# utiasASRL/mm_masking

Hardware: AMD Instinct MI355X
Metric: scan-pairs/s (mask-CNN + 10-iter dICP fwd+bwd) (higher is better)
Workload: dtype bf16; 1 GPU; BASELINE configs[2]: train_icp_weights step fwd+bwd, batch=32 per GPU, 10 dICP iters, point-to-plane Huber, dim=2; 400x3360 polar radar -> GO-CFAR + peaks + polar->Cartesian 640x640 -> U-Net (hand-written NHWC bf16 MFMA kernels, fp32 masters) -> dICP (fp32 points, fp64 normal equations) -> rot+trans+mask_pts loss -> Adam; batch_per_gpu=32, global_batch=32, scan_pts_pad=5120, map_pts=20000, map_pts_pad=20480, icp_iters=10, parallelism=dp1, scene_density=survey (SURVEY.md 8d: 3 500-5 000 valid scan points of 5 120)

## Files before the change

include/mmk.h:

```cpp
#ifndef MMK_H_
#define MMK_H_

#include <stddef.h>
#include <stdint.h>

#ifdef __cplusplus
extern "C" {
#endif

#define MMK_VERSION 502

#define MMK_OK 0
#define MMK_ERR_ARG (-1)
#define MMK_ERR_HIP (-2)
#define MMK_ERR_WORKSPACE (-3)

#define MMK_ICP_PT2PT 0
#define MMK_ICP_PT2PL 1

#define MMK_NN_BRUTE 0
#define MMK_NN_GRID 1

#define MMK_LOSS_NONE 0
#define MMK_LOSS_CAUCHY 1
// ... 72 lines not shown
int mmk_pose_loss_fwd(const float *T_pred , int32_t B, float *out2, void *stream);
int mmk_pose_loss_bwd(const float *T_pred, int32_t B, const float *g_rot, const float *g_trans,
                      float *grad_T , void *stream);
size_t mmk_bce_ws_bytes(void);
int mmk_bce_mean_fwd(const float *x, const float *target, int64_t n, void *ws, size_t ws_bytes,
                     float *out, void *stream);
int mmk_bce_mean_bwd(const float *x, const float *target, int64_t n, const float *grad_out,
                     float *grad_x, void *stream);

int mmk_pose_loss_gt_fwd(const float *T_pred , const float *T_gt , int32_t B, float *out2, void *stream);
int mmk_pose_loss_gt_bwd(const float *T_pred, const float *T_gt, int32_t B, const float *g_rot, const float *g_trans,
                         float *grad_T , void *stream);
int mmk_val_metric(const float *T_pred , const float *T_gt , int32_t B, float *out3, void *stream);
size_t mmk_fft_threshold_ws_bytes(int32_t B);
int mmk_fft_threshold_mask(const float *fft, int32_t B, int64_t hw, void *ws, size_t ws_bytes, float *mask_out,
                           void *stream);
int mmk_bce_fft_threshold_fwd(const float *x, const float *fft, int32_t B, int64_t hw, void *ws, size_t ws_bytes,
                              float *thr_out , float *out, void *stream);
int mmk_bce_fft_threshold_bwd(const float *x, const float *fft, int32_t B, int64_t hw, const float *thr ,
                              const float *grad_out, float *grad_x, void *stream);


int mmk_cfar_mask(const float *raw, int32_t B, int32_t A, int32_t R, int32_t w2,
                  int32_t guard, int32_t mincol, int32_t maxcol, float a_thresh,
                  float b_thresh, int32_t diff, float steep_fact, float *mask,
                  void *stream);

int mmk_cfar_mask_bwd(const float *raw, const float *grad_mask , int32_t B, int32_t A, int32_t R, int32_t w2,
                      int32_t guard, int32_t mincol, int32_t maxcol, float a_thresh, float b_thresh, float steep_fact,
                      float *grad_raw , void *stream);

size_t mmk_extract_peaks_workspace_bytes(int32_t B, int32_t A, int32_t R, int32_t max_pts);
int mmk_extract_peaks(const float *mask, int32_t B, int32_t A, int32_t R, float res,
                      const float *azimuths , const float *times ,
                      const float *T_ab, int32_t diff, float steep_fact, int32_t max_pts,
                      float *out_pc, int32_t *out_count, void *workspace,
                      size_t workspace_bytes, void *stream);
size_t mmk_extract_peaks_bwd_workspace_bytes(int32_t B, int32_t A, int32_t R, int32_t max_pts);
int mmk_extract_peaks_bwd(const float *mask, int32_t B, int32_t A, int32_t R, float res, const float *azimuths ,
                          const float *T_ab, int32_t diff, float steep_fact, int32_t max_pts,
                          const float *grad_pc , float *grad_mask , void *workspace,
                          size_t workspace_bytes, void *stream);

int mmk_polar_to_cart(const float *polar, const float *azimuths ,
                      const float *range_grid, const float *angle_grid, int32_t B,
                      int32_t A, int32_t R, int32_t W, float radar_resolution,
                      int32_t interpolate_crossover, int32_t fix_wobble, float *cart,
                      void *stream);
int mmk_polar_to_cart_pair(const float *polar, const float *polar2, const float *azimuths,
                           const float *range_grid, const float *angle_grid, int32_t B, int32_t A,
                           int32_t R, int32_t W, float radar_resolution, int32_t interpolate_crossover,
                           int32_t fix_wobble, float *cart, float *cart2, void *stream);

int mmk_cart_to_polar(const double *cart, const double *sin_az, const double *cos_az, const double *range_coords,
                      int32_t B, int32_t A, int32_t R, int32_t H, int32_t W, double cart_resolution, double *polar,
                      void *stream);

size_t mmk_polar_to_cart_bwd_ws_bytes(int32_t B, int32_t A, int32_t R, int32_t W);
int mmk_polar_to_cart_bwd(const float *grad_cart , const float *azimuths , const float *range_grid,
                          const float *angle_grid, int32_t B, int32_t A, int32_t R, int32_t W, float radar_resolution,
                          int32_t interpolate_crossover, int32_t fix_wobble, float *grad_polar , void *ws,
                          size_t ws_bytes, void *stream);

size_t mmk_cart_to_polar_bwd_ws_bytes(int32_t B, int32_t A, int32_t R, int32_t H, int32_t W);
int mmk_cart_to_polar_bwd(const double *grad_polar , const double *sin_az, const double *cos_az,
                          const double *range_coords, int32_t B, int32_t A, int32_t R, int32_t H, int32_t W,
                          double radar_resolution, double cart_resolution, double *grad_cart , void *ws,
                          size_t ws_bytes, void *stream);

int mmk_mask_polar_scan(const float *scan , const float *mask_cart , const double *sin_az,
                        const double *cos_az, const double *range_coords, int32_t B, int32_t A, int32_t R, int32_t H,
                        int32_t W, double cart_resolution, float *out , void *stream);

size_t mmk_mask_polar_scan_bwd_ws_bytes(int32_t B, int32_t A, int32_t R, int32_t H, int32_t W);
int mmk_mask_polar_scan_bwd(const float *grad_out , const float *scan , const float *mask_cart ,
                            const double *sin_az, const double *cos_az, const double *range_coords, int32_t B, int32_t A,
                            int32_t R, int32_t H, int32_t W, double radar_resolution, double cart_resolution,
                            float *grad_scan , float *grad_mask , void *ws, size_t ws_bytes,
                            void *stream);

int mmk_sample_weights_fwd(const float *mask , const float *pc ,
                           int32_t B, int32_t N, int32_t pc_cols, int32_t H, int32_t W,
                           int32_t cart_pixel_width, float cart_resolution,
                           float *weights , void *stream);
size_t mmk_sample_weights_bwd_ws_bytes(int32_t B, int32_t N);
int mmk_sample_weights_bwd(const float *grad_weights , const float *pc, int32_t B,
                           int32_t N, int32_t pc_cols, int32_t H, int32_t W,
                           int32_t cart_pixel_width, float cart_resolution, float *grad_mask,
                           void *ws, size_t ws_bytes, void *stream);
int mmk_sample_weights_bwd_pc(const float *grad_weights , const float *mask , const float *pc,
                              int32_t B, int32_t N, int32_t pc_cols, int32_t H, int32_t W,
                              int32_t cart_pixel_width, float cart_resolution, float *grad_pc, void *stream);

int mmk_host_read_rows(const char *path, int64_t header_bytes, int32_t rows, int32_t row_bytes, int32_t col0,
                       int32_t ncols, int32_t roll, void *dst);
typedef struct mmk_read_job {
    const char *path;
    int64_t header_bytes;
    int32_t rows, row_bytes, col0, ncols, roll, reserved;
    void *dst;
} mmk_read_job;
int mmk_host_read_rows_batch(const mmk_read_job *jobs, int32_t n_jobs, int32_t threads);
int mmk_u8_to_float(const void *in , const float *lut256, int64_t n, float *out, void *stream);

int mmk_weight_stats(const float *weights , const float *pc , int32_t B, int32_t N,
                     int32_t pc_cols, float *partial, float *out, void *stream);

int mmk_bev_raster(const float *pc , int32_t B, int32_t M, int32_t pc_cols,
                   int32_t W, float cart_resolution, float *bev , void *stream);

typedef struct {
    const void *x1;
    const void *x2;
    int32_t C1, C2;
    const void *wpack;
    const float *bias;
    void *y1;
    const void *relu_src1;
    int32_t O1, accumulate1;
    float scale1;
    void *y2;
    const void *relu_src2;
    int32_t O2, accumulate2;
    float scale2;
    int32_t B, H, W;
    int32_t relu;
    float leaky_slope;
    float drop_p;
    uint32_t seed;
    void *pool_y;
    void *pool_arg;
} mmk_conv_desc;

int32_t mmk_conv3x3_pool_fusable(int32_t cin, int32_t cout, int32_t B, int32_t H, int32_t W);

size_t mmk_conv3x3_packed_elems(int32_t cout, int32_t cin, int32_t transposed);
int mmk_conv3x3_pack_weights(const float *W, int32_t cout, int32_t cin, int32_t transposed,
                             void *packed, void *stream);
int mmk_conv3x3_pack_weights_batch(int32_t n, const float *const *W, const int32_t *cout, const int32_t *cin,
                                   int32_t transposed, void *const *packed, void *stream);
int mmk_conv3x3(const mmk_conv_desc *d, void *stream);
int32_t mmk_conv3x3_wgrad_slices(int32_t cout, int32_t cin, int32_t c1, int32_t B, int32_t H, int32_t W);
int mmk_conv3x3_wgrad_partial(const void *x1, const void *x2, int32_t C1, int32_t C2, const void *g, int32_t cout,
                              int32_t B, int32_t H, int32_t W, float *partials, int32_t accumulate, void *stream);

int mmk_conv_bwd_fused(const void *x, const void *g, const void *wpack_t, float scale, int32_t B, int32_t H, int32_t W,
                       int32_t C, void *dx, float *partials, int32_t accumulate, void *stream);

int mmk_conv8x16_bwd_fused(const void *x, const void *g, const void *wpack_t, float scale, int32_t B, int32_t H, int32_t W,
                           void *dx, float *partials, int32_t accumulate, void *stream);

int mmk_conv16x8_bwd_fused(const void *x1, const void *x2, const void *g, const void *wpack_t, float scale, int32_t B, int32_t H,
                           int32_t W, void *dx1, void *dx2, float *partials, int32_t accumulate, void *stream);
int mmk_conv3x3_wgrad_unpack_batch(int32_t n, const float *const *src, const int32_t *slices, const int32_t *cout,
                                   const int32_t *cin, float *const *dW, float *const *db, void *stream);

int mmk_channel_minmax(const float *x , int32_t B, int32_t C, int64_t hw, float *part,
                       float *pre , float *minmax , void *stream);
int mmk_channel_meanstd(const float *x , int32_t B, int32_t C, int64_t hw, double *part,
                        float *pre , void *stream);
int mmk_conv_first(const float *x, int32_t cin, const float *W, const float *bias, const float *pre,
                   int32_t B, int32_t H, int32_t Wd, float leaky_slope, void *y, void *stream);
size_t mmk_conv_first_wgrad_ws_bytes(int32_t cin);
int mmk_conv_first_wgrad(const float *x, int32_t cin, const void *g, const float *pre, int32_t B,
                         int32_t H, int32_t Wd, float *dW, float *db, float *ws, size_t ws_bytes, void *stream);
#define MMK_NORM_NONE 0
#define MMK_NORM_MINMAX 1
#define MMK_NORM_STANDARDIZE 2
size_t mmk_conv_first_dgrad_ws_bytes(int32_t cin);
int mmk_conv_first_dgrad(const void *g, int32_t cin, const float *W, const float *x , const float *pre ,
                         const float *minmax , int32_t B, int32_t H, int32_t Wd, float *grad_x, void *ws ,
                         size_t ws_bytes, void *stream);
int mmk_input_norm_bwd(float *grad_x, const float *x, int32_t cin, const float *pre, const float *minmax ,
                       int32_t mode, int32_t B, int32_t H, int32_t Wd, const void *ws, size_t ws_bytes, void *stream);

int mmk_maxpool2_fwd(const void *x, int32_t B, int32_t H, int32_t W, int32_t C, void *y, void *stream);
int mmk_maxpool2_bwd(const void *d, const void *gy, int32_t B, int32_t H, int32_t W, int32_t C, float scale,
                     float leaky_slope, void *gz, void *stream);
int mmk_maxpool2_fwd_arg(const void *x, int32_t B, int32_t H, int32_t W, int32_t C, void *y, void *arg, void *stream);
int mmk_maxpool2_bwd_arg(const void *arg, const void *gy, int32_t B, int32_t H, int32_t W, int32_t C, float scale,
                         void *gz, void *stream);

int mmk_upsample_fwd(const void *x, int32_t B, int32_t Hs, int32_t Ws, int32_t C, int32_t Ho, int32_t Wo, void *y,
                     void *stream);
int mmk_upsample_bwd(const void *gy, int32_t B, int32_t Hs, int32_t Ws, int32_t C, int32_t Ho, int32_t Wo,
                     const void *relu_src, float scale, float leaky_slope, void *gx, void *stream);

#define MMK_FINAL_BWD_WS_FLOATS 16384
int mmk_final_fwd(const void *x, const float *w, const float *bias, int64_t npix, float *mask, void *stream);
int mmk_final_bwd(const void *x, const float *w, const float *mask, const float *gmask, int64_t npix, float scale,
                  float leaky_slope, void *gx, float *dW, float *db, float *ws, void *stream);
int mmk_mask_normalize(const float *mask , int32_t B, int64_t npix_per, float *part,
                       float *mask_n, float *amax, void *stream);
int mmk_final_bwd_normalized(const void *x, const float *w, const float *mask, const float *mask_n,
                             const float *amax, const float *gmask_n, int32_t B, int64_t npix_per,
                             float scale, float leaky_slope, float *part, float *coef, void *gx, float *dW,
                             float *db, float *ws, void *stream);

int mmk_bn_forward_stats(const void *a, int64_t npix, int32_t C, const float *gamma, const float *beta, float eps,
                         float momentum, float *running_mean, float *running_var, float *part, float *stat,
                         float *affine, void *stream);
int mmk_bn_apply(const void *a, int64_t npix, int32_t C, const float *affine, float drop_p, uint32_t seed, void *y,
                 void *stream);
int mmk_bn_backward(const void *gd, const void *d, float drop_scale, const void *a, int64_t npix, int32_t C,
                    const float *stat, const float *affine, const float *gamma, float leaky_slope, int32_t accumulate,
                    float *part, float *coef, float *dgamma, float *dbeta, void *gz, void *stream);

typedef struct {
    int32_t B, H, W, cin;
    const float *x;
    const float *pre;
    const float *const *params;
    float drop_p;
    uint32_t seed;
    float leaky_slope;
    int32_t norm;
    void *workspace;
    size_t workspace_bytes;
    float *mask;
    int32_t keep_full_res;
} mmk_unet_desc;

size_t mmk_unet_workspace_bytes(int32_t B, int32_t H, int32_t W, int32_t cin);
size_t mmk_unet_scratch_bytes(int32_t B, int32_t H, int32_t W, int32_t cin);
int mmk_unet_forward(const mmk_unet_desc *d, void *stream);
int mmk_unet_backward(const mmk_unet_desc *d, const float *gmask, float *const *grads, void *scratch,
                      size_t scratch_bytes, void *stream);
#define MMK_UNET_GRAD_BUCKETS 3
int32_t mmk_unet_grad_bucket(int32_t bucket, int32_t *first_param, int32_t *n_params);
int mmk_unet_backward_buckets(const mmk_unet_desc *d, const float *gmask, float *const *grads, void *scratch,
                              size_t scratch_bytes, void *const *bucket_events, void *stream);
int mmk_unet_backward_input(const mmk_unet_desc *d, const float *gmask, float *const *grads, float *grad_x, int32_t norm_mode,
                            const float *minmax, void *scratch, size_t scratch_bytes, void *const *bucket_events, void *stream);
int mmk_unet_tensor(int32_t B, int32_t H, int32_t W, int32_t cin, int32_t id, size_t *offset, int32_t *h,
                    int32_t *w, int32_t *c);

#ifdef __cplusplus
}
#endif
#endif
```

mm_masking_amd/_lib.py:

```python
import ctypes
import os
import sys
import subprocess

import torch

_HERE = os.path.dirname(os.path.abspath(__file__))
_ROOT = os.path.dirname(_HERE)
SO_PATH = os.environ.get("MMK_LIB", os.path.join(_HERE, "libmmk_hip.so"))
SOURCES = ["mmk_api.hip", "mmk_icp.hip", "mmk_radar.hip", "mmk_unet.hip", "mmk_unet_driver.hip", "mmk_loader.hip", "mmk_loss.hip"]

_lib = None

c_f32p = ctypes.c_void_p
c_vp = ctypes.c_void_p


class MmkError(RuntimeError):
    pass


class ReadJob(ctypes.Structure):
    _fields_ = [("path", ctypes.c_char_p), ("header_bytes", ctypes.c_int64), ("rows", ctypes.c_int32),
                ("row_bytes", ctypes.c_int32), ("col0", ctypes.c_int32), ("ncols", ctypes.c_int32), ("roll", ctypes.c_int32),
                ("reserved", ctypes.c_int32), ("dst", ctypes.c_void_p)]


class IcpParams(ctypes.Structure):
    _fields_ = [("B", ctypes.c_int32), ("N", ctypes.c_int32), ("M", ctypes.c_int32),
                ("tgt_cols", ctypes.c_int32), ("dim", ctypes.c_int32), ("icp_type", ctypes.c_int32),
                ("loss", ctypes.c_int32), ("loss_k", ctypes.c_float), ("trim_dist", ctypes.c_float),
                ("tolerance", ctypes.c_float), ("max_iter", ctypes.c_int32), ("save_state", ctypes.c_int32),
                ("check_every", ctypes.c_int32), ("nn_method", ctypes.c_int32)]


class ConvDesc(ctypes.Structure):
    _fields_ = [("x1", ctypes.c_void_p), ("x2", ctypes.c_void_p), ("C1", ctypes.c_int32), ("C2", ctypes.c_int32),
                ("wpack", ctypes.c_void_p), ("bias", ctypes.c_void_p),
                ("y1", ctypes.c_void_p), ("relu_src1", ctypes.c_void_p), ("O1", ctypes.c_int32),
                ("accumulate1", ctypes.c_int32), ("scale1", ctypes.c_float),
                ("y2", ctypes.c_void_p), ("relu_src2", ctypes.c_void_p), ("O2", ctypes.c_int32),
                ("accumulate2", ctypes.c_int32), ("scale2", ctypes.c_float),
                ("B", ctypes.c_int32), ("H", ctypes.c_int32), ("W", ctypes.c_int32), ("relu", ctypes.c_int32),
                ("leaky_slope", ctypes.c_float), ("drop_p", ctypes.c_float), ("seed", ctypes.c_uint32), ("pool_y", ctypes.c_void_p),
                ("pool_arg", ctypes.c_void_p)]


class UNetDesc(ctypes.Structure):
    _fields_ = [("B", ctypes.c_int32), ("H", ctypes.c_int32), ("W", ctypes.c_int32), ("cin", ctypes.c_int32),
                ("x", ctypes.c_void_p), ("pre", ctypes.c_void_p), ("params", ctypes.POINTER(ctypes.c_void_p)),
                ("drop_p", ctypes.c_float), ("seed", ctypes.c_uint32), ("leaky_slope", ctypes.c_float), ("norm", ctypes.c_int32),
                ("workspace", ctypes.c_void_p), ("workspace_bytes", ctypes.c_size_t), ("mask", ctypes.c_void_p),
                ("keep_full_res", ctypes.c_int32)]


FINAL_BWD_WS_FLOATS = 16384
NORM_MODES = {None: 0, "none": 0, "minmax": 1, "standardize": 2}
ICP_TYPES = {"pt2pt": 0, "pt2pl": 1}
LOSSES = {None: 0, "none": 0, "l2": 0, "cauchy": 1, "huber": 2}
NN_METHODS = {"brute": 0, "grid": 1}


def build(verbose=False):
    from concurrent.futures import ThreadPoolExecutor
    csrc = os.path.join(_HERE, "csrc")
    srcs = [os.path.join(csrc, s) for s in SOURCES]
    common = [os.path.join(csrc, "mmk_common.h"), os.path.join(csrc, "mmk_unet_shared.h"), os.path.join(_ROOT, "include", "mmk.h")]
    incs = [os.path.join(csrc, f) for f in sorted(os.listdir(csrc)) if f.endswith(".inc")]
    extra = {"mmk_unet.hip": incs, "mmk_loader.hip": incs}
    objdir = os.path.join(csrc, "_obj")
    os.makedirs(objdir, exist_ok=True)
    hipcc = os.environ.get("HIPCC", "/opt/rocm/bin/hipcc")
    flags = ["--offload-arch=gfx950", "-O3", "-std=c++17", "-fPIC", "-ffp-contract=off", "-I", os.path.join(_ROOT, "include")]
    per_file = {"mmk_unet.hip": ["-mllvm", "-amdgpu-mfma-vgpr-form"]}
    jobs, objs = [], []
    for src in srcs:
        obj = os.path.join(objdir, os.path.basename(src)[:-4] + ".o")
        objs.append(obj)
        deps = [src] + common + extra.get(os.path.basename(src), []) + [os.path.abspath(__file__)]
        if not (os.path.exists(obj) and all(os.path.getmtime(obj) >= os.path.getmtime(d) for d in deps)):
            jobs.append([hipcc] + flags + per_file.get(os.path.basename(src), []) + ["-c", src, "-o", obj])
    if not jobs and os.path.exists(SO_PATH) and all(os.path.getmtime(SO_PATH) >= os.path.getmtime(o) for o in objs):
        return SO_PATH

    def run(cmd):
        if verbose:
            print(" ".join(cmd), flush=True)
        try:
            subprocess.check_call(cmd)
        except subprocess.CalledProcessError:
            plain = [c for c in cmd if c not in sum(per_file.values(), [])]
            if len(plain) == len(cmd):
                raise
            print("libmmk_hip: retrying without %s" % " ".join(sorted(set(cmd) - set(plain))), file=sys.stderr, flush=True)
            subprocess.check_call(plain)
    with ThreadPoolExecutor(max_workers=max(1, min(len(jobs), os.cpu_count() or 1))) as ex:
        list(ex.map(run, jobs))
    run([hipcc, "--offload-arch=gfx950", "-shared", "-fPIC", "-o", SO_PATH] + objs)
    return SO_PATH


def _declare(lib):
    i32, f32, sz = ctypes.c_int32, ctypes.c_float, ctypes.c_size_t
    P = ctypes.POINTER(IcpParams)
    sig = {
        "mmk_version": (ctypes.c_int, []),
        "mmk_last_error": (ctypes.c_char_p, []),
        "mmk_icp_workspace_bytes": (sz, [P]),
        "mmk_icp_forward": (ctypes.c_int, [P] + [c_vp] * 10 + [c_vp, sz, ctypes.POINTER(ctypes.c_int), c_vp]),
        "mmk_icp_backward": (ctypes.c_int, [P] + [c_vp] * 11 + [c_vp, sz, c_vp]),
        "mmk_icp_backward_points_workspace_bytes": (sz, [P, i32]),
        "mmk_icp_backward_points": (ctypes.c_int, [P] + [c_vp] * 13 + [c_vp, sz, c_vp]),
        "mmk_icp_status": (ctypes.c_int, [P, c_vp, sz, c_vp, c_vp]),
        "mmk_pose_loss_fwd": (ctypes.c_int, [c_vp, i32, c_vp, c_vp]),
        "mmk_pose_loss_bwd": (ctypes.c_int, [c_vp, i32, c_vp, c_vp, c_vp, c_vp]),
        "mmk_bce_ws_bytes": (sz, []),
        "mmk_bce_mean_fwd": (ctypes.c_int, [c_vp, c_vp, ctypes.c_int64, c_vp, sz, c_vp, c_vp]),
        "mmk_bce_mean_bwd": (ctypes.c_int, [c_vp, c_vp, ctypes.c_int64, c_vp, c_vp, c_vp]),
        "mmk_pose_loss_gt_fwd": (ctypes.c_int, [c_vp, c_vp, i32, c_vp, c_vp]),
        "mmk_pose_loss_gt_bwd": (ctypes.c_int, [c_vp, c_vp, i32, c_vp, c_vp, c_vp, c_vp]),
        "mmk_val_metric": (ctypes.c_int, [c_vp, c_vp, i32, c_vp, c_vp]),
        "mmk_fft_threshold_ws_bytes": (sz, [i32]),
        "mmk_fft_threshold_mask": (ctypes.c_int, [c_vp, i32, ctypes.c_int64, c_vp, sz, c_vp, c_vp]),
        "mmk_bce_fft_threshold_fwd": (ctypes.c_int, [c_vp, c_vp, i32, ctypes.c_int64, c_vp, sz, c_vp, c_vp, c_vp]),
        "mmk_bce_fft_threshold_bwd": (ctypes.c_int, [c_vp, c_vp, i32, ctypes.c_int64, c_vp, c_vp, c_vp, c_vp]),
        "mmk_icp_partials_count": (sz, [P]),
        "mmk_icp_accumulate": (ctypes.c_int, [P] + [c_vp] * 8 + [c_vp]),
        "mmk_icp_solve_update": (ctypes.c_int, [P] + [c_vp] * 7 + [c_vp]),
        "mmk_nn_padded_m": (i32, [i32]),
        "mmk_pack_target": (ctypes.c_int, [c_vp, i32, i32, i32, i32, c_vp, c_vp]),
        "mmk_nn_workspace_bytes": (sz, [i32, i32, i32, i32]),
        "mmk_nn_search": (ctypes.c_int, [c_vp, c_vp, c_vp, i32, i32, i32, i32, c_vp, c_vp, c_vp, sz, c_vp]),
        "mmk_nn_profile_begin": (ctypes.c_int, [i32]),
        "mmk_nn_profile_end": (ctypes.c_int, [ctypes.POINTER(ctypes.c_float), i32, ctypes.POINTER(ctypes.c_int32)]),
        "mmk_conv3x3_packed_elems": (sz, [i32, i32, i32]),
        "mmk_conv3x3_pack_weights": (ctypes.c_int, [c_vp, i32, i32, i32, c_vp, c_vp]),
        "mmk_conv3x3_pack_weights_batch": (ctypes.c_int, [i32, c_vp, c_vp, c_vp, i32, c_vp, c_vp]),
        "mmk_conv3x3": (ctypes.c_int, [ctypes.POINTER(ConvDesc), c_vp]),
        "mmk_conv3x3_wgrad_unpack_batch": (ctypes.c_int, [i32, c_vp, c_vp, c_vp, c_vp, c_vp, c_vp, c_vp]),
        "mmk_conv3x3_wgrad_slices": (i32, [i32, i32, i32, i32, i32, i32]),
        "mmk_conv3x3_wgrad_partial": (ctypes.c_int, [c_vp, c_vp, i32, i32, c_vp, i32, i32, i32, i32, c_vp, i32, c_vp]),
        "mmk_conv_bwd_fused": (ctypes.c_int, [c_vp, c_vp, c_vp, ctypes.c_float, i32, i32, i32, i32, c_vp, c_vp, i32, c_vp]),
        "mmk_conv8x16_bwd_fused": (ctypes.c_int, [c_vp, c_vp, c_vp, ctypes.c_float, i32, i32, i32, c_vp, c_vp, i32, c_vp]),
        "mmk_conv16x8_bwd_fused": (ctypes.c_int, [c_vp, c_vp, c_vp, c_vp, ctypes.c_float, i32, i32, i32, c_vp, c_vp, c_vp, i32, c_vp]),
        "mmk_conv3x3_pool_fusable": (ctypes.c_int32, [i32, i32, i32, i32, i32]),
        "mmk_channel_minmax": (ctypes.c_int, [c_vp, i32, i32, ctypes.c_int64, c_vp, c_vp, c_vp, c_vp]),
        "mmk_channel_meanstd": (ctypes.c_int, [c_vp, i32, i32, ctypes.c_int64, c_vp, c_vp, c_vp]),
        "mmk_conv_first": (ctypes.c_int, [c_vp, i32, c_vp, c_vp, c_vp, i32, i32, i32, f32, c_vp, c_vp]),
        "mmk_conv_first_wgrad_ws_bytes": (sz, [i32]),
        "mmk_conv_first_wgrad": (ctypes.c_int, [c_vp, i32, c_vp, c_vp, i32, i32, i32, c_vp, c_vp, c_vp, sz, c_vp]),
        "mmk_conv_first_dgrad_ws_bytes": (sz, [i32]),
        "mmk_conv_first_dgrad": (ctypes.c_int, [c_vp, i32, c_vp, c_vp, c_vp, c_vp, i32, i32, i32, c_vp, c_vp, sz, c_vp]),
        "mmk_input_norm_bwd": (ctypes.c_int, [c_vp, c_vp, i32, c_vp, c_vp, i32, i32, i32, i32, c_vp, sz, c_vp]),
        "mmk_maxpool2_fwd": (ctypes.c_int, [c_vp, i32, i32, i32, i32, c_vp, c_vp]),
        "mmk_maxpool2_bwd": (ctypes.c_int, [c_vp, c_vp, i32, i32, i32, i32, f32, f32, c_vp, c_vp]),
        "mmk_maxpool2_fwd_arg": (ctypes.c_int, [c_vp, i32, i32, i32, i32, c_vp, c_vp, c_vp]),
        "mmk_maxpool2_bwd_arg": (ctypes.c_int, [c_vp, c_vp, i32, i32, i32, i32, f32, c_vp, c_vp]),
        "mmk_upsample_fwd": (ctypes.c_int, [c_vp, i32, i32, i32, i32, i32, i32, c_vp, c_vp]),
        "mmk_upsample_bwd": (ctypes.c_int, [c_vp, i32, i32, i32, i32, i32, i32, c_vp, f32, f32, c_vp, c_vp]),
        "mmk_final_fwd": (ctypes.c_int, [c_vp, c_vp, c_vp, ctypes.c_int64, c_vp, c_vp]),
        "mmk_final_bwd": (ctypes.c_int, [c_vp, c_vp, c_vp, c_vp, ctypes.c_int64, f32, f32, c_vp, c_vp, c_vp, c_vp, c_vp]),
        "mmk_mask_normalize": (ctypes.c_int, [c_vp, i32, ctypes.c_int64, c_vp, c_vp, c_vp, c_vp]),
        "mmk_final_bwd_normalized": (ctypes.c_int, [c_vp, c_vp, c_vp, c_vp, c_vp, c_vp, i32, ctypes.c_int64, f32, f32, c_vp, c_vp,
                                                    c_vp, c_vp, c_vp, c_vp, c_vp]),
        "mmk_bn_forward_stats": (ctypes.c_int, [c_vp, ctypes.c_int64, i32, c_vp, c_vp, f32, f32, c_vp, c_vp, c_vp, c_vp, c_vp, c_vp]),
        "mmk_bn_apply": (ctypes.c_int, [c_vp, ctypes.c_int64, i32, c_vp, f32, ctypes.c_uint32, c_vp, c_vp]),
        "mmk_bn_backward": (ctypes.c_int, [c_vp, c_vp, f32, c_vp, ctypes.c_int64, i32, c_vp, c_vp, c_vp, f32, i32, c_vp, c_vp, c_vp,
                                           c_vp, c_vp, c_vp]),
        "mmk_unet_workspace_bytes": (sz, [i32, i32, i32, i32]),
        "mmk_unet_scratch_bytes": (sz, [i32, i32, i32, i32]),
        "mmk_unet_forward": (ctypes.c_int, [ctypes.POINTER(UNetDesc), c_vp]),
        "mmk_unet_backward": (ctypes.c_int, [ctypes.POINTER(UNetDesc), c_vp, ctypes.POINTER(ctypes.c_void_p), c_vp, sz, c_vp]),
        "mmk_unet_backward_buckets": (ctypes.c_int, [ctypes.POINTER(UNetDesc), c_vp, ctypes.POINTER(ctypes.c_void_p), c_vp, sz,
                                                     ctypes.POINTER(ctypes.c_void_p), c_vp]),
        "mmk_unet_backward_input": (ctypes.c_int, [ctypes.POINTER(UNetDesc), c_vp, ctypes.POINTER(ctypes.c_void_p), c_vp, i32, c_vp,
                                                   c_vp, sz, ctypes.POINTER(ctypes.c_void_p), c_vp]),
        "mmk_unet_grad_bucket": (i32, [i32, ctypes.POINTER(i32), ctypes.POINTER(i32)]),
        "mmk_unet_tensor": (ctypes.c_int, [i32, i32, i32, i32, i32, ctypes.POINTER(sz), ctypes.POINTER(i32), ctypes.POINTER(i32),
                                           ctypes.POINTER(i32)]),
        "mmk_cfar_mask": (ctypes.c_int, [c_vp, i32, i32, i32, i32, i32, i32, i32, f32, f32, i32, f32, c_vp, c_vp]),
        "mmk_cfar_mask_bwd": (ctypes.c_int, [c_vp, c_vp, i32, i32, i32, i32, i32, i32, i32, f32, f32, f32, c_vp, c_vp]),
        "mmk_extract_peaks_workspace_bytes": (sz, [i32, i32, i32, i32]),
        "mmk_extract_peaks_bwd_workspace_bytes": (sz, [i32, i32, i32, i32]),
        "mmk_extract_peaks_bwd": (ctypes.c_int, [c_vp, i32, i32, i32, f32, c_vp, c_vp, i32, f32, i32, c_vp, c_vp, c_vp, sz, c_vp]),
        "mmk_extract_peaks": (ctypes.c_int, [c_vp, i32, i32, i32, f32, c_vp, c_vp, c_vp, i32, f32, i32, c_vp, c_vp,
                                             c_vp, sz, c_vp]),
        "mmk_polar_to_cart": (ctypes.c_int, [c_vp, c_vp, c_vp, c_vp, i32, i32, i32, i32, f32, i32, i32, c_vp, c_vp]),
        "mmk_polar_to_cart_pair": (ctypes.c_int, [c_vp, c_vp, c_vp, c_vp, c_vp, i32, i32, i32, i32, f32, i32, i32, c_vp, c_vp,
                                                  c_vp]),
        "mmk_cart_to_polar": (ctypes.c_int, [c_vp, c_vp, c_vp, c_vp, i32, i32, i32, i32, i32, ctypes.c_double, c_vp, c_vp]),
        "mmk_polar_to_cart_bwd_ws_bytes": (sz, [i32, i32, i32, i32]),
        "mmk_polar_to_cart_bwd": (ctypes.c_int, [c_vp, c_vp, c_vp, c_vp, i32, i32, i32, i32, f32, i32, i32, c_vp, c_vp, sz, c_vp]),
        "mmk_cart_to_polar_bwd_ws_bytes": (sz, [i32, i32, i32, i32, i32]),
        "mmk_cart_to_polar_bwd": (ctypes.c_int, [c_vp, c_vp, c_vp, c_vp, i32, i32, i32, i32, i32, ctypes.c_double, ctypes.c_double,
                                                 c_vp, c_vp, sz, c_vp]),
        "mmk_mask_polar_scan": (ctypes.c_int, [c_vp, c_vp, c_vp, c_vp, c_vp, i32, i32, i32, i32, i32, ctypes.c_double, c_vp, c_vp]),
        "mmk_mask_polar_scan_bwd_ws_bytes": (sz, [i32, i32, i32, i32, i32]),
        "mmk_mask_polar_scan_bwd": (ctypes.c_int, [c_vp, c_vp, c_vp, c_vp, c_vp, c_vp, i32, i32, i32, i32, i32, ctypes.c_double,
                                                   ctypes.c_double, c_vp, c_vp, c_vp, sz, c_vp]),
        "mmk_sample_weights_fwd": (ctypes.c_int, [c_vp, c_vp, i32, i32, i32, i32, i32, i32, f32, c_vp, c_vp]),
        "mmk_host_read_rows": (ctypes.c_int, [ctypes.c_char_p, ctypes.c_int64, i32, i32, i32, i32, i32, c_vp]),
        "mmk_host_read_rows_batch": (ctypes.c_int, [ctypes.POINTER(ReadJob), i32, i32]),
        "mmk_u8_to_float": (ctypes.c_int, [c_vp, c_vp, ctypes.c_int64, c_vp, c_vp]),
        "mmk_sample_weights_bwd_ws_bytes": (sz, [i32, i32]),
        "mmk_sample_weights_bwd": (ctypes.c_int, [c_vp, c_vp, i32, i32, i32, i32, i32, i32, f32, c_vp, c_vp, sz, c_vp]),
        "mmk_sample_weights_bwd_pc": (ctypes.c_int, [c_vp, c_vp, c_vp, i32, i32, i32, i32, i32, i32, f32, c_vp, c_vp]),
        "mmk_weight_stats": (ctypes.c_int, [c_vp, c_vp, i32, i32, i32, c_vp, c_vp, c_vp]),
        "mmk_bev_raster": (ctypes.c_int, [c_vp, i32, i32, i32, i32, f32, c_vp, c_vp]),
    }
    for name, (res, args) in sig.items():
        fn = getattr(lib, name)
        fn.restype = res
        fn.argtypes = args
    return sig


EXPORTED = None


def lib():
    global _lib, EXPORTED
    if _lib is None:
        if not os.path.exists(SO_PATH):
            raise MmkError("libmmk_hip.so is not built: run `python -c 'import __graft_entry__ as g; g.build()'` "
                           "(hipcc --offload-arch=gfx950).  The HIP path has no CPU fallback.")
        try:
            loaded = ctypes.CDLL(SO_PATH)
        except OSError as e:
            raise MmkError("cannot load %s: %s" % (SO_PATH, e)) from e
        EXPORTED = _declare(loaded)
        _lib = loaded
    return _lib


def check(rc):
    if rc != 0:
        raise MmkError("libmmk_hip: %s (code %d)" % (lib().mmk_last_error().decode(errors="replace"), rc))


def stream_ptr(device=None):
    if device is not None:
        idx = device.index if isinstance(device, torch.device) else int(device)
        if idx is not None and idx != torch.cuda.current_device():
            raise MmkError("tensors live on cuda:%d but the current HIP device is cuda:%d: call torch.cuda.set_device() "
                           "(one process per GPU) or wrap the call in `with torch.cuda.device(...)`"
                           % (idx, torch.cuda.current_device()))
    return ctypes.c_void_p(torch.cuda.current_stream(device).cuda_stream)


def ptr(t, dtype=None, name="tensor"):
    if t is None:
        return ctypes.c_void_p(0)
    if not t.is_cuda:
        raise MmkError("%s must live on a HIP device (got %s); the kernels have no CPU path" % (name, t.device))
    if dtype is not None and t.dtype != dtype:
        raise MmkError("%s must be %s (got %s)" % (name, dtype, t.dtype))
    if not t.is_contiguous():
        raise MmkError("%s must be contiguous" % name)
    return ctypes.c_void_p(t.data_ptr())


def dev_f32(t, device):
    return t.detach().to(device=device, dtype=torch.float32).contiguous()
```

mm_masking_amd/csrc/mmk_unet.hip:

```cpp
#include <math.h>
#include <stdlib.h>

#include <algorithm>
#include <type_traits>

#include "mmk_common.h"
#include "mmk_unet_shared.h"

namespace {

using namespace mmku;

__device__ __forceinline__ unsigned cvt_pk_bf16(float lo, float hi)
{
    unsigned r;
    asm("v_cvt_pk_bf16_f32 %0, %1, %2" : "=v"(r) : "v"(lo), "v"(hi));
    return r;
}
__device__ __forceinline__ unsigned pk_relu_bf16(unsigned x)
{
    unsigned r;
    asm("v_pk_max_i16 %0, %1, 0" : "=v"(r) : "v"(x));
    return r;
}
// ... 1419 lines not shown
        t_end = min(total_tiles, (xcd + 1) * per_xcd);
    } else {
        t_first = blockIdx.x; t_step = gridDim.x; t_end = total_tiles;
    }
    const int adv_tx = t_step % tiles_x, adv_ty = (t_step / tiles_x) % tiles_y, adv_b = t_step / tpi;
    int ld_b = t_first / tpi, ld_ty = (t_first % tpi) / tiles_x, ld_tx = t_first % tiles_x;
    if (t_first < t_end) load_tile(ld_b, ld_ty, ld_tx);
    for (int t = t_first; t < t_end; t += t_step) {
        __syncthreads();
        store_tile();
        __syncthreads();
        {
            if (t + t_step < t_end) {
                ld_tx += adv_tx;
                const int cx = ld_tx >= tiles_x ? 1 : 0;
                ld_tx -= cx ? tiles_x : 0;
                ld_ty += adv_ty + cx;
                const int cy = ld_ty >= tiles_y ? 1 : 0;
                ld_ty -= cy ? tiles_y : 0;
                ld_b += adv_b + cy;
            }
            load_tile(ld_b, ld_ty, ld_tx);
        }
        i32x2 fa[2][2 * MT], fb[2][2 * NTW];
#define WG_ISSUE(R, BUF)                                                                                 \
    {                                                                                                    \
        _Pragma("unroll") for (int m = 0; m < MT; ++m) {                                                 \
            fa[BUF][2 * m] = (m == 0) ? tr_read_o<((R) * TW * PG) * 2>(g_ad)                             \
                           : (m == 1) ? tr_read_o<((R) * TW * PG + 16) * 2>(g_ad)                        \
                           : (m == 2) ? tr_read_o<((R) * TW * PG + 32) * 2>(g_ad)                        \
                                      : tr_read_o<((R) * TW * PG + 48) * 2>(g_ad);                       \
            fa[BUF][2 * m + 1] = (m == 0) ? tr_read_o<((R) * TW * PG + 16 * PG) * 2>(g_ad)                \
                               : (m == 1) ? tr_read_o<((R) * TW * PG + 16 + 16 * PG) * 2>(g_ad)           \
                               : (m == 2) ? tr_read_o<((R) * TW * PG + 32 + 16 * PG) * 2>(g_ad)           \
                                          : tr_read_o<((R) * TW * PG + 48 + 16 * PG) * 2>(g_ad);          \
        }                                                                                                \
        _Pragma("unroll") for (int n = 0; n < NTW; ++n) {                                                \
            fb[BUF][2 * n] = tr_read_o<((R) * WT * PK) * 2>(b_ad[n]);                                    \
            fb[BUF][2 * n + 1] = tr_read_o<((R) * WT * PK + 16 * PK) * 2>(b_ad[n]);                       \
        }                                                                                                \
    }
#define WG_CONSUME(BUF)                                                                                  \
    {                                                                                                    \
        _Pragma("unroll") for (int m = 0; m < MT; ++m) {                                                 \
            const bf16x8 af = frag_from(fa[BUF][2 * m], fa[BUF][2 * m + 1]);                             \
             \
             \
            _Pragma("unroll") for (int n = 0; n < NTW; ++n)                                              \
                acc[m][n] = __builtin_amdgcn_mfma_f32_16x16x32_bf16(af, frag_from(fb[BUF][2 * n], fb[BUF][2 * n + 1]), acc[m][n], 0, 0, 0); \
            accb[m] = __builtin_amdgcn_mfma_f32_16x16x32_bf16(af, ones, accb[m], 0, 0, 0);               \
        }                                                                                                \
    }
#define WG_STEP(R)                                                                                       \
    {                                                                                                    \
        asm volatile("s_waitcnt lgkmcnt(0)" ::: "memory");                                               \
        __builtin_amdgcn_sched_barrier(0);                                                               \
        if ((R) + 1 < TH) WG_ISSUE(((R) + 1 < TH ? (R) + 1 : 0), ((R) + 1) & 1);                         \
        __builtin_amdgcn_sched_barrier(0);                                                               \
        WG_CONSUME((R) & 1);                                                                             \
    }
        WG_ISSUE(0, 0);
        WG_STEP(0) WG_STEP(1) WG_STEP(2) WG_STEP(3) WG_STEP(4) WG_STEP(5) WG_STEP(6) WG_STEP(7)
        static_assert(TH == 8, "WG_STEP expansion above covers 8 tile rows");
#undef WG_STEP
#undef WG_CONSUME
#undef WG_ISSUE
    }

    const size_t pstride = (size_t)9 * a.COUT * a.CIN + a.COUT;
#pragma unroll
    for (int m = 0; m < MT; ++m) {
#pragma unroll
        for (int rr = 0; rr < 4; ++rr) {
            const int co = group * CM + m * 16 + g4 * 4 + rr;
            if (co >= a.COUT) continue;
#pragma unroll
            for (int n = 0; n < NTW; ++n) {
                const int nt = wv + 4 * n;
                if (nt >= NTT) continue;
                int tap, ci;
                if (CK >= 16) {
                    tap = nt / (CK / 16);
                    ci = chunk * CK + (nt % (CK / 16)) * 16 + i16;
                } else {
                    tap = 2 * nt + (i16 >> 3);
                    ci = i16 & 7;
                }
                if (tap < 9) {
                    float *d = a.partials + (size_t)blockIdx.x * pstride + ((size_t)tap * a.COUT + co) * a.CIN + ci;
                    *d = a.acc_partials ? *d + acc[m][n][rr] : acc[m][n][rr];
                }
            }
            if (wv == 0 && chunk == 0 && i16 == 0) {
                float *d = a.partials + (size_t)blockIdx.x * pstride + (size_t)9 * a.COUT * a.CIN + co;
                *d = a.acc_partials ? *d + accb[m][rr] : accb[m][rr];
            }
        }
    }
}

template <int CK, int CM, bool G8>
int wgrad_spatial(int cout, int cin, int B, int H, int W)
{
    const size_t smem = ((size_t)(HT * WT + 8) * wg_pitch(CK) + (size_t)(TH * TW + 8) * wg_pitch(G8 ? 8 : CM)) * sizeof(bf16);
    static int per_cu[64] = {};
    int dev = 0;
    if (hipGetDevice(&dev) != hipSuccess) return -1;
    if (per_cu[dev & 63] == 0) {
        if (smem > 64 * 1024 &&
            hipFuncSetAttribute((const void *)conv3x3_wgrad_kernel<CK, CM, G8>, hipFuncAttributeMaxDynamicSharedMemorySize, (int)smem) != hipSuccess)
            return -1;
        int nblk = 0;
        if (hipOccupancyMaxActiveBlocksPerMultiprocessor(&nblk, conv3x3_wgrad_kernel<CK, CM, G8>, CONV_THREADS, smem) != hipSuccess)
            return -1;
        const int cap = (CK <= 16 && CM == 16) ? 4 : 8;
        per_cu[dev & 63] = nblk < 1 ? 1 : (nblk > cap ? cap : nblk);
    }
    const int tiles = ((W + TW - 1) / TW) * ((H + TH - 1) / TH) * B;
    const int chunks = cin / CK, groups = (cout + CM - 1) / CM;
    int spatial = (256 * per_cu[dev & 63]) / (chunks * groups);
    spatial = spatial < 1 ? 1 : (spatial > tiles ? tiles : spatial);
    return spatial >= 8 ? (spatial & ~7) : spatial;
}

template <int CK, int CM, bool G8>
int launch_wgrad(const WgradArgs &a, hipStream_t st)
{
    const size_t smem = ((size_t)(HT * WT + 8) * wg_pitch(CK) + (size_t)(TH * TW + 8) * wg_pitch(G8 ? 8 : CM)) * sizeof(bf16);
    const int spatial = wgrad_spatial<CK, CM, G8>(a.COUT, a.CIN, a.B, a.H, a.W);
    if (spatial < 1) {
        mmk::set_error("mmk_conv3x3_wgrad: occupancy query failed");
        return MMK_ERR_HIP;
    }
    const int chunks = a.CIN / CK, groups = (a.COUT + CM - 1) / CM;
    hipLaunchKernelGGL((conv3x3_wgrad_kernel<CK, CM, G8>), dim3(spatial, chunks, groups), dim3(CONV_THREADS), smem, st, a);
    MMK_LAUNCH_CHECK();
    return MMK_OK;
}


struct BwdFusedArgs {
    const bf16 *x, *x2;
    const bf16 *g;
    const bf16 *wpack_t;
    bf16 *dx, *dx2;
    float scale;
    int masked;
    int accumulate_dx;
    int B, H, W;
    float *partials;
    int acc_partials;
};

template <int CX, int CG>
__global__ __launch_bounds__(CONV_THREADS) void conv_bwd_fused_kernel(const BwdFusedArgs a)
{
    static_assert((CX == 8 || CX == 16) && (CG == 8 || CG == 16), "thin layers");
    constexpr int NTT = CX == 8 ? 5 : 9;
    constexpr int NTW = (NTT + 3) / 4;
    constexpr int NS = CG == 8 ? 3 : 5;
    constexpr int NT = 4;
    constexpr int GX = CX / 8, GG = CG / 8;
    __shared__ __attribute__((aligned(16))) bf16 x_tile[(HT * WT + 8) * CX];
    __shared__ __attribute__((aligned(16))) bf16 g_tile[(HT * WT + 8) * CG];
    __shared__ __attribute__((aligned(16))) bf16 w_lds[NS * 64 * 8];

    const int tid = threadIdx.x, lane = tid & 63;
    const int wv = __builtin_amdgcn_readfirstlane(tid >> 6);
    const int tiles_x = (a.W + TW - 1) / TW, tiles_y = (a.H + TH - 1) / TH;
    const int tpi = tiles_x * tiles_y;
    const int total_tiles = tpi * a.B;
    const int i16 = lane & 15, g4 = lane >> 4, q = i16 >> 2, pp = i16 & 3;
    const bool split = a.x2 != nullptr;

    f32x4 acc[NTW], accb = {0.f, 0.f, 0.f, 0.f};
#pragma unroll
    for (int n = 0; n < NTW; ++n) acc[n] = (f32x4){0.f, 0.f, 0.f, 0.f};
    bf16x8 ones;
#pragma unroll
    for (int j = 0; j < 8; ++j) ones[j] = (bf16)1.0f;
    unsigned b_ad[NTW];
#pragma unroll
    for (int n = 0; n < NTW; ++n) {
        const int nt = wv + 4 * n;
        int tap = CX == 8 ? 2 * nt + (pp >> 1) : nt;
        const int col = CX == 8 ? 4 * (pp & 1) : 4 * pp;
        tap = tap > 8 ? 8 : tap;
        const int ty = tap / 3, tx = tap % 3;
        b_ad[n] = lds_addr(x_tile) + (unsigned)((((ty * WT) + 4 * g4 + q + tx) * CX + col) * 2);
    }
    const unsigned g_ad = lds_addr(g_tile) + (unsigned)(((WT + 1 + 4 * g4 + q) * CG + 4 * pp) * 2);

    int d_lane[NS];
#pragma unroll
    for (int ks = 0; ks < NS; ++ks) {
        int tap = CG == 8 ? 4 * ks + (lane >> 4) : 2 * ks + (lane >> 5);
        const int ch = CG == 8 ? 0 : 8 * ((lane >> 4) & 1);
        tap = tap > 8 ? 8 : tap;
        d_lane[ks] = ((2 * wv + tap / 3) * WT + (lane & 15) + tap % 3) * CG + ch;
    }
    const int n8 = lane >> 4;
    const int lrow8 = 2 * wv + (n8 >> 1), lcol8 = (n8 & 1) * 16 + (lane & 15);
    const int lpix8 = lrow8 * a.W + lcol8;
    const int s_off8 = ((lrow8 + 1) * WT + lcol8 + 1) * CX;
    int o_pix[NT], s_off[NT];
#pragma unroll
    for (int n = 0; n < NT; ++n) {
        const int r = 2 * wv + (n >> 1), c = (n & 1) * 16 + (lane & 15);
        o_pix[n] = r * a.W + c;
        s_off[n] = ((r + 1) * WT + c + 1) * CX + (lane >> 4) * 4;
    }
    bf16 *const o_base = (a.dx2 != nullptr) ? ((lane >> 5) ? a.dx2 : a.dx) + ((lane >> 4) & 1) * 4 : a.dx + (lane >> 4) * 4;
    const int o_stride = (a.dx2 != nullptr) ? 8 : 16;
    for (int i = tid; i < NS * 64; i += CONV_THREADS) reinterpret_cast<u32x4 *>(w_lds)[i] = reinterpret_cast<const u32x4 *>(a.wpack_t)[i];

    constexpr int NX = HT * WT * GX, NG = HT * WT * GG;
    constexpr int RX = (NX + CONV_THREADS - 1) / CONV_THREADS, RG = (NG + CONV_THREADS - 1) / CONV_THREADS;
    u32x4 rx[RX], rg[RG];
    auto load_tile = [&](int b, int tyi, int txi) {
        int tv = tid;
        asm volatile("" : "+v"(tv));
        const int tx0 = txi * TW, ty0 = tyi * TH;
        const int pix0 = (b * a.H + ty0) * a.W + tx0;
#pragma unroll
        for (int i = 0; i < RX; ++i) {
            int gi = tv + i * CONV_THREADS;
            gi = gi < NX ? gi : NX - 1;
            const int pix = gi / GX, half = gi % GX;
            const int dy = pix / WT - 1, dx = pix % WT - 1;
            const bool ok = (unsigned)(ty0 + dy) < (unsigned)a.H && (unsigned)(tx0 + dx) < (unsigned)a.W;
            const long po = pix0 + dy * a.W + dx;
            const bf16 *src = split ? (half ? a.x2 : a.x) + po * 8 : a.x + po * CX + half * 8;
            rx[i] = *(ok ? reinterpret_cast<const u32x4 *>(src) : &g_zero16);
        }
#pragma unroll
        for (int i = 0; i < RG; ++i) {
            int gi = tv + i * CONV_THREADS;
            gi = gi < NG ? gi : NG - 1;
            const int pix = gi / GG, gc = gi % GG;
            const int dy = pix / WT - 1, dx = pix % WT - 1;
            const bool ok = (unsigned)(ty0 + dy) < (unsigned)a.H && (unsigned)(tx0 + dx) < (unsigned)a.W;
            rg[i] = *(ok ? reinterpret_cast<const u32x4 *>(a.g + (long)(pix0 + dy * a.W + dx) * CG + gc * 8) : &g_zero16);
        }
    };
    auto store_tile = [&]() {
        int tv = tid;
        asm volatile("" : "+v"(tv));
#pragma unroll
        for (int i = 0; i < RX; ++i) {
            const int gi = tv + i * CONV_THREADS;
            if (gi < NX) *reinterpret_cast<u32x4 *>(x_tile + (size_t)gi * 8) = rx[i];
        }
#pragma unroll
        for (int i = 0; i < RG; ++i) {
            const int gi = tv + i * CONV_THREADS;
            if (gi < NG) *reinterpret_cast<u32x4 *>(g_tile + (size_t)gi * 8) = rg[i];
        }
    };

    int t_first, t_step, t_end;
    if ((gridDim.x & 7) == 0) {
        const int per_xcd = (total_tiles + 7) / 8;
        const int xcd = blockIdx.x & 7;
        t_first = xcd * per_xcd + ((int)blockIdx.x >> 3);
        t_step = (int)gridDim.x >> 3;
        t_end = min(total_tiles, (xcd + 1) * per_xcd);
    } else {
        t_first = blockIdx.x; t_step = gridDim.x; t_end = total_tiles;
    }
    const int adv_tx = t_step % tiles_x, adv_ty = (t_step / tiles_x) % tiles_y, adv_b = t_step / tpi;
    int ld_b = t_first / tpi, ld_ty = (t_first % tpi) / tiles_x, ld_tx = t_first % tiles_x;
    int cb = ld_b, cty = ld_ty, ctx = ld_tx;
    if (t_first < t_end) {
        load_tile(ld_b, ld_ty, ld_tx);
        store_tile();
    }
    __syncthreads();
    for (int t = t_first; t < t_end; t += t_step) {
        const int b = cb;
        const int tx0 = ctx * TW, ty0 = cty * TH;
        const int pix0 = (b * a.H + ty0) * a.W + tx0;
        const bool ok8 = (ty0 + lrow8) < a.H && (tx0 + lcol8) < a.W;
        u32x4 e8_acc = {0u, 0u, 0u, 0u};
        if constexpr (CX == 8) e8_acc = *((ok8 && a.accumulate_dx) ? reinterpret_cast<const u32x4 *>(a.dx + (long)(pix0 + lpix8) * 8) : &g_zero16);
        {
            if (t + t_step < t_end) {
                ld_tx += adv_tx;
                const int cx = ld_tx >= tiles_x ? 1 : 0;
                ld_tx -= cx ? tiles_x : 0;
                ld_ty += adv_ty + cx;
                const int cy = ld_ty >= tiles_y ? 1 : 0;
                ld_ty -= cy ? tiles_y : 0;
                ld_b += adv_b + cy;
            }
            load_tile(ld_b, ld_ty, ld_tx);
            cb = ld_b; cty = ld_ty; ctx = ld_tx;
        }
        i32x2 fa[2][2], fb[2][2 * NTW];
#define BF_ISSUE(R, BUF)                                                                     \
    {                                                                                        \
        fa[BUF][0] = tr_read_o<((R) * WT * CG) * 2>(g_ad);                                   \
        fa[BUF][1] = tr_read_o<((R) * WT * CG + 16 * CG) * 2>(g_ad);                         \
        _Pragma("unroll") for (int n = 0; n < NTW; ++n) {                                    \
            fb[BUF][2 * n] = tr_read_o<((R) * WT * CX) * 2>(b_ad[n]);                        \
            fb[BUF][2 * n + 1] = tr_read_o<((R) * WT * CX + 16 * CX) * 2>(b_ad[n]);          \
        }                                                                                    \
    }
#define BF_CONSUME(BUF)                                                                      \
    {                                                                                        \
        const bf16x8 af = frag_from(fa[BUF][0], fa[BUF][1]);                                 \
        _Pragma("unroll") for (int n = 0; n < NTW; ++n)                                      \
            acc[n] = __builtin_amdgcn_mfma_f32_16x16x32_bf16(af, frag_from(fb[BUF][2 * n], fb[BUF][2 * n + 1]), acc[n], 0, 0, 0); \
        accb = __builtin_amdgcn_mfma_f32_16x16x32_bf16(af, ones, accb, 0, 0, 0);             \
    }
#define BF_STEP(R)                                                                           \
    {                                                                                        \
        asm volatile("s_waitcnt lgkmcnt(0)" ::: "memory");                                   \
        __builtin_amdgcn_sched_barrier(0);                                                   \
        if ((R) + 1 < TH) BF_ISSUE(((R) + 1 < TH ? (R) + 1 : 0), ((R) + 1) & 1);             \
        __builtin_amdgcn_sched_barrier(0);                                                   \
        BF_CONSUME((R) & 1);                                                                 \
    }
        BF_ISSUE(0, 0);
        BF_STEP(0) BF_STEP(1) BF_STEP(2) BF_STEP(3) BF_STEP(4) BF_STEP(5) BF_STEP(6) BF_STEP(7)
        static_assert(TH == 8, "BF_STEP expansion above covers 8 tile rows");
#undef BF_STEP
#undef BF_CONSUME
#undef BF_ISSUE
        f32x4 dacc[NT];
#pragma unroll
        for (int n = 0; n < NT; ++n) dacc[n] = (f32x4){0.f, 0.f, 0.f, 0.f};
#pragma unroll
        for (int ks = 0; ks < NS; ++ks) {
            const bf16 *bl = g_tile + d_lane[ks];
            bf16x8 bf[NT];
#pragma unroll
            for (int n = 0; n < NT; ++n) bf[n] = *reinterpret_cast<const bf16x8 *>(bl + ((n >> 1) * WT + (n & 1) * 16) * CG);
            const bf16x8 af = *reinterpret_cast<const bf16x8 *>(w_lds + ((size_t)(ks * 64 + lane)) * 8);
#pragma unroll
            for (int n = 0; n < NT; ++n) dacc[n] = __builtin_amdgcn_mfma_f32_16x16x32_bf16(af, bf[n], dacc[n], 0, 0, 0);
        }
        u32x4 e8_src = {0u, 0u, 0u, 0u};
        bf16x4 e_src[NT];
        if constexpr (CX == 8) {
            e8_src = *reinterpret_cast<const u32x4 *>(x_tile + s_off8);
        } else {
#pragma unroll
            for (int n = 0; n < NT; ++n) e_src[n] = *reinterpret_cast<const bf16x4 *>(x_tile + s_off[n]);
        }
#pragma unroll
        for (int i = 0; i < RX; ++i) asm volatile("" : "+v"(rx[i]));
#pragma unroll
        for (int i = 0; i < RG; ++i) asm volatile("" : "+v"(rg[i]));
        if constexpr (CX == 8) {
            float v8[8];
#pragma unroll
            for (int r = 0; r < 4; ++r) {
                const auto s01 = __builtin_amdgcn_permlane16_swap(__float_as_uint(dacc[0][r]), __float_as_uint(dacc[1][r]), false, false);
                const auto s23 = __builtin_amdgcn_permlane16_swap(__float_as_uint(dacc[2][r]), __float_as_uint(dacc[3][r]), false, false);
                const auto lo = __builtin_amdgcn_permlane32_swap(s01[0], s23[0], false, false);
                const auto hi = __builtin_amdgcn_permlane32_swap(s01[1], s23[1], false, false);
                v8[r] = __uint_as_float(lo[0]);
                v8[4 + r] = __uint_as_float(hi[0]);
            }
            float sv[8], av[8];
            unpack8(e8_src, sv);
            unpack8(e8_acc, av);
#pragma unroll
            for (int r = 0; r < 8; ++r) {
                const float v = fmaxf(v8[r] + 0.f, -INFINITY);
                const float masked = (sv[r] > 0.f) ? v * a.scale : 0.f;
                v8[r] = masked + av[r];
            }
            u32x4 *dst8 = ok8 ? reinterpret_cast<u32x4 *>(a.dx + (long)(pix0 + lpix8) * 8) : reinterpret_cast<u32x4 *>(g_sink16);
            *dst8 = pack8(v8);
        } else {
#pragma unroll
            for (int n = 0; n < NT; ++n) {
                const bool okp = (ty0 + 2 * wv + (n >> 1)) < a.H && (tx0 + (n & 1) * 16 + (lane & 15)) < a.W;
                bf16x4 outv;
#pragma unroll
                for (int r = 0; r < 4; ++r) {
                    const float v = fmaxf(dacc[n][r] + 0.f, -INFINITY);
                    const float masked = ((float)e_src[n][r] > 0.f) ? v * a.scale : 0.f;
                    outv[r] = (bf16)(a.masked ? masked + 0.f : v);
                }
                bf16x4 *dst = okp ? reinterpret_cast<bf16x4 *>(o_base + (long)(pix0 + o_pix[n]) * o_stride) : reinterpret_cast<bf16x4 *>(g_sink16);
                *dst = outv;
            }
        }
        if (t + t_step >= t_end) break;
        __syncthreads();
        store_tile();
        __syncthreads();
    }

    constexpr size_t pstride = (size_t)9 * CG * CX + CG;
#pragma unroll
    for (int rr = 0; rr < 4; ++rr) {
        const int co = g4 * 4 + rr;
        if (co >= CG) continue;
#pragma unroll
        for (int n = 0; n < NTW; ++n) {
            const int nt = wv + 4 * n;
            if (nt >= NTT) continue;
            const int tap = CX == 8 ? 2 * nt + (i16 >> 3) : nt;
            const int ci = CX == 8 ? (i16 & 7) : i16;
            if (tap < 9) {
                float *d = a.partials + (size_t)blockIdx.x * pstride + ((size_t)tap * CG + co) * CX + ci;
                *d = a.acc_partials ? *d + acc[n][rr] : acc[n][rr];
            }
        }
        if (wv == 0 && i16 == 0) {
            float *d = a.partials + (size_t)blockIdx.x * pstride + (size_t)9 * CG * CX + co;
            *d = a.acc_partials ? *d + accb[rr] : accb[rr];
        }
    }
}

constexpr int WGD_THREADS = 512;

__global__ __launch_bounds__(WGD_THREADS) void conv3x3_wgrad_deep_kernel(const WgradArgs a)
{
    constexpr int CK = 64, CM = 64, PK = wg_pitch(64), PG = wg_pitch(64);
    extern __shared__ __attribute__((aligned(16))) unsigned char smem[];
    bf16 *x_tile = reinterpret_cast<bf16 *>(smem);
    bf16 *g_tile = x_tile + (HT * WT + 8) * PK;

    const int tid = threadIdx.x, lane = tid & 63;
    const int wv = __builtin_amdgcn_readfirstlane(tid >> 6);
    const int wm = wv >> 2, wc = wv & 3;
    const int chunk = blockIdx.y, group = blockIdx.z;
    const int tiles_x = (a.W + TW - 1) / TW, tiles_y = (a.H + TH - 1) / TH;
    const int tpi = tiles_x * tiles_y;
    const int total_tiles = tpi * a.B;
    const int i16 = lane & 15, g4 = lane >> 4, q = i16 >> 2, pp = i16 & 3;

    f32x4 acc[3][3][2];
    f32x4 accb[2];
#pragma unroll
    for (int m = 0; m < 2; ++m) {
        accb[m] = (f32x4){0.f, 0.f, 0.f, 0.f};
#pragma unroll
        for (int ty = 0; ty < 3; ++ty)
#pragma unroll
            for (int tx = 0; tx < 3; ++tx) acc[ty][tx][m] = (f32x4){0.f, 0.f, 0.f, 0.f};
    }
    bf16x8 ones;
#pragma unroll
    for (int j = 0; j < 8; ++j) ones[j] = (bf16)1.0f;

    const unsigned xb0 = lds_addr(x_tile) + (unsigned)(((4 * g4 + q) * PK + wc * 16 + 4 * pp) * 2);
    const unsigned gb0 = lds_addr(g_tile) + (unsigned)(((4 * g4 + q) * PG + wm * 32 + 4 * pp) * 2);

    constexpr int GPP = CK / 8;
    constexpr int NIN = HT * WT * GPP;
    constexpr int RIN = (NIN + WGD_THREADS - 1) / WGD_THREADS;
    constexpr int GPG = CM / 8;
    constexpr int NG = TH * TW * GPG;
    constexpr int RG = (NG + WGD_THREADS - 1) / WGD_THREADS;
    u32x4 rin[RIN], rg[RG];
    auto load_tile = [&](int b, int tyi, int txi) {
        int tv = tid;
        asm volatile("" : "+v"(tv));
        const int tx0 = txi * TW, ty0 = tyi * TH;
        const int c0 = chunk * CK;
        const bool in1 = c0 < a.C1;
        const bf16 *xb = in1 ? a.x1 : a.x2;
        const int xc = in1 ? a.C1 : a.C2, cb = in1 ? c0 : c0 - a.C1;
#pragma unroll
        for (int i = 0; i < RIN; ++i) {
            int gi = tv + i * WGD_THREADS;
            gi = gi < NIN ? gi : NIN - 1;
            const int pix = gi / GPP, gc = gi % GPP;
            const int yy = ty0 + pix / WT - 1, xx = tx0 + pix % WT - 1;
            const bool ok = yy >= 0 && yy < a.H && xx >= 0 && xx < a.W;
            const size_t p = ((size_t)b * a.H + yy) * a.W + xx;
            const u32x4 *sp = ok ? reinterpret_cast<const u32x4 *>(xb + p * xc + cb + gc * 8) : &g_zero16;
            rin[i] = *sp;
        }
#pragma unroll
        for (int i = 0; i < RG; ++i) {
            int gi = tv + i * WGD_THREADS;
            gi = gi < NG ? gi : NG - 1;
            const int pix = gi / GPG, gc = gi % GPG;
            const int yy = ty0 + pix / TW, xx = tx0 + pix % TW;
            const bool ok = yy < a.H && xx < a.W;
            const size_t p = ((size_t)b * a.H + yy) * a.W + xx;
            const u32x4 *sp = ok ? reinterpret_cast<const u32x4 *>(a.g + p * a.COUT + group * CM + gc * 8) : &g_zero16;
            rg[i] = *sp;
        }
    };
    auto store_tile = [&]() {
        int tv = tid;
        asm volatile("" : "+v"(tv));
#pragma unroll
        for (int i = 0; i < RIN; ++i) {
            const int gi = tv + i * WGD_THREADS;
            if (gi < NIN) *reinterpret_cast<u32x4 *>(x_tile + (size_t)(gi / GPP) * PK + (gi % GPP) * 8) = rin[i];
        }
#pragma unroll
        for (int i = 0; i < RG; ++i) {
            const int gi = tv + i * WGD_THREADS;
            if (gi < NG) *reinterpret_cast<u32x4 *>(g_tile + (size_t)(gi / GPG) * PG + (gi % GPG) * 8) = rg[i];
        }
    };

    int t_first, t_step, t_end;
    if ((gridDim.x & 7) == 0) {
        const int per_xcd = (total_tiles + 7) / 8;
        const int xcd = blockIdx.x & 7;
        t_first = xcd * per_xcd + ((int)blockIdx.x >> 3);
        t_step = (int)gridDim.x >> 3;
        t_end = min(total_tiles, (xcd + 1) * per_xcd);
    } else {
        t_first = blockIdx.x; t_step = gridDim.x; t_end = total_tiles;
    }
    const int adv_tx = t_step % tiles_x, adv_ty = (t_step / tiles_x) % tiles_y, adv_b = t_step / tpi;
    int ld_b = t_first / tpi, ld_ty = (t_first % tpi) / tiles_x, ld_tx = t_first % tiles_x;
    if (t_first < t_end) load_tile(ld_b, ld_ty, ld_tx);
    for (int t = t_first; t < t_end; t += t_step) {
        __syncthreads();
        store_tile();
        __syncthreads();
        {
            if (t + t_step < t_end) {
                ld_tx += adv_tx;
                const int cx = ld_tx >= tiles_x ? 1 : 0;
                ld_tx -= cx ? tiles_x : 0;
                ld_ty += adv_ty + cx;
                const int cy = ld_ty >= tiles_y ? 1 : 0;
                ld_ty -= cy ? tiles_y : 0;
                ld_b += adv_b + cy;
            }
            load_tile(ld_b, ld_ty, ld_tx);
        }
        i32x2 fb[2][3][2], fa[4][2][2];
#define WGD_ISSUE(RHO)                                                                                   \
    {                                                                                                    \
        fb[(RHO) & 1][0][0] = tr_read_o<(((RHO) * WT + 0) * PK) * 2>(xb0);                               \
        fb[(RHO) & 1][0][1] = tr_read_o<(((RHO) * WT + 0) * PK + 16 * PK) * 2>(xb0);                     \
        fb[(RHO) & 1][1][0] = tr_read_o<(((RHO) * WT + 1) * PK) * 2>(xb0);                               \
        fb[(RHO) & 1][1][1] = tr_read_o<(((RHO) * WT + 1) * PK + 16 * PK) * 2>(xb0);                     \
        fb[(RHO) & 1][2][0] = tr_read_o<(((RHO) * WT + 2) * PK) * 2>(xb0);                               \
        fb[(RHO) & 1][2][1] = tr_read_o<(((RHO) * WT + 2) * PK + 16 * PK) * 2>(xb0);                     \
        if ((RHO) < TH) {                                                                                \
            constexpr int R_ = (RHO) < TH ? (RHO) : 0;                                                   \
            fa[R_ & 3][0][0] = tr_read_o<((R_ * TW) * PG) * 2>(gb0);                                     \
            fa[R_ & 3][0][1] = tr_read_o<((R_ * TW) * PG + 16 * PG) * 2>(gb0);                           \
            fa[R_ & 3][1][0] = tr_read_o<((R_ * TW) * PG + 16) * 2>(gb0);                                \
            fa[R_ & 3][1][1] = tr_read_o<((R_ * TW) * PG + 16 + 16 * PG) * 2>(gb0);                      \
        }                                                                                                \
    }
#define WGD_STEP(RHO)                                                                                    \
    {                                                                                                    \
        asm volatile("s_waitcnt lgkmcnt(0)" ::: "memory");                                               \
        __builtin_amdgcn_sched_barrier(0);                                                               \
                                          \
        if ((RHO) + 1 < HT) WGD_ISSUE(((RHO) + 1 < HT ? (RHO) + 1 : 0));                                 \
        __builtin_amdgcn_sched_barrier(0);                                                               \
        bf16x8 bfr[3];                                                                                   \
        _Pragma("unroll") for (int tx = 0; tx < 3; ++tx) bfr[tx] = frag_from(fb[(RHO) & 1][tx][0], fb[(RHO) & 1][tx][1]); \
        _Pragma("unroll") for (int ty = 0; ty < 3; ++ty) {                                               \
            const int r = (RHO) - ty;                \
            if (r >= 0 && r < TH) {                                                                      \
                _Pragma("unroll") for (int m = 0; m < 2; ++m) {                                          \
                    const bf16x8 af = frag_from(fa[r & 3][m][0], fa[r & 3][m][1]);                       \
                    _Pragma("unroll") for (int tx = 0; tx < 3; ++tx)                                     \
// ... 1468 lines not shown
    const int c = blockIdx.x * blockDim.x + threadIdx.x;
    if (c < C) coef[3 * c] = affine[2 * c];
}

__global__ __launch_bounds__(256) void bn_bwd_apply_kernel(const bf16 *__restrict__ gd, const bf16 *__restrict__ d, float drop_scale,
                                                           const bf16 *__restrict__ a, size_t ngran, int C,
                                                           const float *__restrict__ stat, const float *__restrict__ coef, float slope,
                                                           bf16 *__restrict__ gz)
{
    const int G = C >> 3;
    for (size_t e = (size_t)blockIdx.x * blockDim.x + threadIdx.x; e < ngran; e += (size_t)gridDim.x * blockDim.x) {
        const int gc = (int)(e % G);
        float g[8], v[8], o[8];
        bn_gy8(gd, d, e * 8, drop_scale, g);
        unpack8(*reinterpret_cast<const u32x4 *>(a + e * 8), v);
#pragma unroll
        for (int j = 0; j < 8; ++j) {
            const int c = gc * 8 + j;
            float ga;
            if (stat != nullptr) {
                const float xh = (v[j] - stat[2 * c]) * stat[2 * c + 1];
                ga = coef[3 * c] * ((g[j] - coef[3 * c + 1]) - xh * coef[3 * c + 2]);
            } else {
                ga = g[j] * coef[3 * c];
            }
            const float f = (slope > 0.f) ? ((v[j] > 0.f) ? 1.f : slope) : ((v[j] > 0.f) ? 1.f : 0.f);
            o[j] = ga * f;
        }
        *reinterpret_cast<u32x4 *>(gz + e * 8) = pack8(o);
    }
}

bool chan_ok(int c) { return c == 8 || c == 16 || c == 32 || (c >= 64 && c % 64 == 0); }

}

#ifdef MMK_DEEP_STAMPS
extern "C" int mmk_debug_deep_stamps(unsigned long long *buf)
{
    MMK_CHECK_HIP(hipMemcpyToSymbol(HIP_SYMBOL(g_deep_stamp_buf), &buf, sizeof(buf)));
    return MMK_OK;
}
#endif

extern "C" size_t mmk_conv3x3_packed_elems(int32_t cout, int32_t cin, int32_t transposed)
{
    const int co_n = transposed ? cin : cout, ci_n = transposed ? cout : cin;
    if (!chan_ok(co_n) || !chan_ok(ci_n)) return 0;
    const int CK = conv_ck(ci_n), CM = conv_cm(ci_n, co_n);
    const int groups = (co_n + CM - 1) / CM, chunks = ci_n / CK;
    return (size_t)groups * chunks * ksteps(CK) * (CM / 16) * 512;
}

extern "C" int mmk_conv3x3_pack_weights(const float *W, int32_t cout, int32_t cin, int32_t transposed, void *packed,
                                        void *stream)
{
    MMK_REQUIRE(W && packed, "mmk_conv3x3_pack_weights: NULL pointer");
    const size_t total = mmk_conv3x3_packed_elems(cout, cin, transposed);
    MMK_REQUIRE(total > 0, "mmk_conv3x3_pack_weights: unsupported channel counts %d -> %d", cin, cout);
    hipLaunchKernelGGL(pack_conv_weights_kernel, dim3((unsigned)((total + 255) / 256)), dim3(256), 0, (hipStream_t)stream, W,
                       cout, cin, transposed, (bf16 *)packed, (int)total);
    MMK_LAUNCH_CHECK();
    return MMK_OK;
}

extern "C" int mmk_conv3x3_pack_weights_batch(int32_t n, const float *const *W, const int32_t *cout, const int32_t *cin,
                                              int32_t transposed, void *const *packed, void *stream)
{
    MMK_REQUIRE(n >= 1 && W && cout && cin && packed, "mmk_conv3x3_pack_weights_batch: bad argument");
    for (int base = 0; base < n; base += PACK_BATCH_MAX) {
        PackBatch pb;
        const int m = std::min(PACK_BATCH_MAX, n - base);
        size_t most = 0;
        for (int i = 0; i < PACK_BATCH_MAX; ++i) {
            const int k = base + (i < m ? i : 0);
            MMK_REQUIRE(W[k] && packed[k], "mmk_conv3x3_pack_weights_batch: NULL pointer (layer %d)", k);
            const size_t total = mmk_conv3x3_packed_elems(cout[k], cin[k], transposed);
            MMK_REQUIRE(total > 0 && total < ((size_t)1 << 31), "mmk_conv3x3_pack_weights_batch: unsupported channel counts %d -> %d",
                        cin[k], cout[k]);
            pb.W[i] = W[k]; pb.out[i] = (bf16 *)packed[k]; pb.cout[i] = cout[k]; pb.cin[i] = cin[k];
            pb.total[i] = (int)total;
            most = std::max(most, total);
        }
        pb.transposed = transposed;
        const unsigned bx = (unsigned)std::min<size_t>((most + 255) / 256, 256);
        hipLaunchKernelGGL(pack_conv_weights_batch_kernel, dim3(bx, m), dim3(256), 0, (hipStream_t)stream, pb);
        MMK_LAUNCH_CHECK();
    }
    return MMK_OK;
}

extern "C" int mmk_conv3x3(const mmk_conv_desc *d, void *stream)
{
    MMK_REQUIRE(d != nullptr, "mmk_conv3x3: NULL descriptor");
    MMK_REQUIRE(d->x1 && d->wpack && (d->y1 || (d->pool_y && d->pool_arg)), "mmk_conv3x3: NULL pointer");
    MMK_REQUIRE(d->pool_arg == nullptr || d->pool_y != nullptr, "mmk_conv3x3: pool_arg needs pool_y");
    MMK_REQUIRE(d->B >= 1 && d->H >= 1 && d->W >= 1, "mmk_conv3x3: bad shape");
    const int cin = d->C1 + d->C2, cout = d->O1 + d->O2;
    MMK_REQUIRE(d->C1 % 8 == 0 && d->C2 % 8 == 0 && (d->C2 == 0 || d->x2), "mmk_conv3x3: bad input split %d+%d", d->C1, d->C2);
    MMK_REQUIRE(d->O1 % 8 == 0 && d->O2 % 8 == 0 && (d->O2 == 0 || d->y2), "mmk_conv3x3: bad output split %d+%d", d->O1, d->O2);
    MMK_REQUIRE(chan_ok(cin) && chan_ok(cout), "mmk_conv3x3: unsupported channel counts %d -> %d", cin, cout);
    MMK_REQUIRE(dropout_prob_ok(d->drop_p), "mmk_conv3x3: dropout probability %g out of range (it is quantised to thr / 65536, thr <= 65535)", (double)d->drop_p);
    ConvArgs a;
    a.x1 = (const bf16 *)d->x1; a.x2 = (const bf16 *)d->x2; a.C1 = d->C1; a.C2 = d->C2;
    a.wpack = (const bf16 *)d->wpack; a.bias = d->bias;
    a.o1 = {(bf16 *)d->y1, (const bf16 *)d->relu_src1, d->O1, d->accumulate1, d->scale1};
    a.o2 = {(bf16 *)d->y2, (const bf16 *)d->relu_src2, d->O2, d->accumulate2, d->scale2};
    a.B = d->B; a.H = d->H; a.W = d->W; a.CIN = cin; a.COUT = cout;
    MMK_REQUIRE(d->leaky_slope >= 0.f && d->leaky_slope <= 1.f, "mmk_conv3x3: leaky_slope must be in [0, 1]");
    a.relu = d->relu; a.slope = d->leaky_slope; a.drop_p = d->drop_p; a.seed = d->seed;
    a.pool_y = (bf16 *)d->pool_y;
    a.pool_arg = (unsigned char *)d->pool_arg;
    return dispatch_conv(a, (hipStream_t)stream);
}

extern "C" int32_t mmk_conv3x3_pool_fusable(int32_t cin, int32_t cout, int32_t B, int32_t H, int32_t W)
{
    return pool_fusable(cin, cout, B, H, W) ? 1 : 0;
}

extern "C" int mmk_conv3x3_wgrad_unpack_batch(int32_t n, const float *const *src, const int32_t *slices, const int32_t *cout,
                                              const int32_t *cin, float *const *dW, float *const *db, void *stream)
{
    MMK_REQUIRE(n >= 1 && src && cout && cin && dW, "mmk_conv3x3_wgrad_unpack_batch: bad argument");
    for (int base = 0; base < n; base += PACK_BATCH_MAX) {
        UnpackBatch ub;
        const int m = std::min(PACK_BATCH_MAX, n - base);
        int most = 0;
        for (int i = 0; i < PACK_BATCH_MAX; ++i) {
            const int k = base + (i < m ? i : 0);
            MMK_REQUIRE(src[k] && dW[k] && cout[k] >= 1 && cin[k] >= 1, "mmk_conv3x3_wgrad_unpack_batch: bad layer %d", k);
            ub.src[i] = src[k]; ub.dW[i] = dW[k]; ub.cout[i] = cout[k]; ub.cin[i] = cin[k];
            ub.slices[i] = slices ? slices[k] : 0;
            ub.db[i] = (db && ub.slices[i] > 0) ? db[k] : nullptr;
            const int total = cout[k] * cin[k] * 9 + (ub.slices[i] > 0 ? cout[k] : 0);
            const int epb = 4 * (256 / unpack_groups(total));
            most = std::max(most, (total + epb - 1) / epb);
        }
        const unsigned bx = (unsigned)std::min(most, 2048);
        hipLaunchKernelGGL(unpack_wgrad_batch_kernel, dim3(bx, m), dim3(256), 0, (hipStream_t)stream, ub);
        MMK_LAUNCH_CHECK();
    }
    return MMK_OK;
}

template <int CX, int CG>
int launch_bwd_fused(const BwdFusedArgs &a, int c1, hipStream_t st)
{
    const int spatial = wgrad_slices(CG, CX, c1, a.B, a.H, a.W);
    if (spatial < 1) {
        mmk::set_error("fused backward: occupancy query failed");
        return MMK_ERR_HIP;
    }
    hipLaunchKernelGGL((conv_bwd_fused_kernel<CX, CG>), dim3(spatial), dim3(CONV_THREADS), 0, st, a);
    MMK_LAUNCH_CHECK();
    return MMK_OK;
}

extern "C" int mmk_conv_bwd_fused(const void *x, const void *g, const void *wpack_t, float scale, int32_t B, int32_t H, int32_t W,
                                  int32_t C, void *dx, float *partials, int32_t accumulate, void *stream)
{
    MMK_REQUIRE(x && g && wpack_t && dx && partials, "mmk_conv_bwd_fused: NULL pointer");
    MMK_REQUIRE(B >= 1 && H >= 2 && W >= 2 && (C == 8 || C == 16), "mmk_conv_bwd_fused: bad shape (8 or 16 channels)");
    MMK_REQUIRE((size_t)B * H * W * C < ((size_t)1 << 31), "mmk_conv_bwd_fused: tensor too large for 32-bit offsets");
    BwdFusedArgs a = {};
    a.x = (const bf16 *)x; a.g = (const bf16 *)g; a.wpack_t = (const bf16 *)wpack_t; a.dx = (bf16 *)dx; a.scale = scale; a.masked = 1;
    a.B = B; a.H = H; a.W = W; a.partials = partials; a.acc_partials = accumulate;
    return C == 8 ? launch_bwd_fused<8, 8>(a, 8, (hipStream_t)stream) : launch_bwd_fused<16, 16>(a, 16, (hipStream_t)stream);
}

extern "C" int mmk_conv8x16_bwd_fused(const void *x, const void *g, const void *wpack_t, float scale, int32_t B, int32_t H, int32_t W,
                                      void *dx, float *partials, int32_t accumulate, void *stream)
{
    MMK_REQUIRE(x && g && wpack_t && dx && partials, "mmk_conv8x16_bwd_fused: NULL pointer");
    MMK_REQUIRE(B >= 1 && H >= 2 && W >= 2, "mmk_conv8x16_bwd_fused: bad shape");
    MMK_REQUIRE((size_t)B * H * W * 16 < ((size_t)1 << 31), "mmk_conv8x16_bwd_fused: tensor too large for 32-bit offsets");
    BwdFusedArgs a = {};
    a.x = (const bf16 *)x; a.g = (const bf16 *)g; a.wpack_t = (const bf16 *)wpack_t; a.dx = (bf16 *)dx; a.scale = scale; a.masked = 1;
    a.accumulate_dx = 1;
    a.B = B; a.H = H; a.W = W; a.partials = partials; a.acc_partials = accumulate;
    return launch_bwd_fused<8, 16>(a, 8, (hipStream_t)stream);
}

extern "C" int mmk_conv16x8_bwd_fused(const void *x1, const void *x2, const void *g, const void *wpack_t, float scale, int32_t B,
                                      int32_t H, int32_t W, void *dx1, void *dx2, float *partials, int32_t accumulate, void *stream)
{
    MMK_REQUIRE(x1 && g && wpack_t && dx1 && partials, "mmk_conv16x8_bwd_fused: NULL pointer");
    MMK_REQUIRE((x2 == nullptr) == (dx2 == nullptr), "mmk_conv16x8_bwd_fused: x2 and dx2 go together (both NULL: one 16-channel input / unmasked output)");
    MMK_REQUIRE(B >= 1 && H >= 2 && W >= 2, "mmk_conv16x8_bwd_fused: bad shape");
    MMK_REQUIRE((size_t)B * H * W * 16 < ((size_t)1 << 31), "mmk_conv16x8_bwd_fused: tensor too large for 32-bit offsets");
    BwdFusedArgs a = {};
    a.x = (const bf16 *)x1; a.x2 = (const bf16 *)x2; a.g = (const bf16 *)g; a.wpack_t = (const bf16 *)wpack_t;
    a.dx = (bf16 *)dx1; a.dx2 = (bf16 *)dx2; a.scale = scale; a.masked = x2 != nullptr;
    a.B = B; a.H = H; a.W = W; a.partials = partials; a.acc_partials = accumulate;
    return launch_bwd_fused<16, 8>(a, x2 ? 8 : 16, (hipStream_t)stream);
}

extern "C" int32_t mmk_conv3x3_wgrad_slices(int32_t cout, int32_t cin, int32_t c1, int32_t B, int32_t H, int32_t W)
{
    if (B < 1 || H < 1 || W < 1 || !chan_ok(cin) || !chan_ok(cout)) return 0;
    const int ns = wgrad_slices(cout, cin, c1, B, H, W);
    return ns < 0 ? 0 : ns;
}

extern "C" int mmk_conv3x3_wgrad_partial(const void *x1, const void *x2, int32_t C1, int32_t C2, const void *g, int32_t cout,
                                         int32_t B, int32_t H, int32_t W, float *partials, int32_t accumulate, void *stream)
{
    MMK_REQUIRE(x1 && g && partials, "mmk_conv3x3_wgrad_partial: NULL pointer");
    MMK_REQUIRE(B >= 1 && H >= 1 && W >= 1, "mmk_conv3x3_wgrad_partial: bad shape");
    const int cin = C1 + C2;
    MMK_REQUIRE(C1 % 8 == 0 && C2 % 8 == 0 && (C2 == 0 || x2), "mmk_conv3x3_wgrad_partial: bad input split %d+%d", C1, C2);
    MMK_REQUIRE(chan_ok(cin) && chan_ok(cout), "mmk_conv3x3_wgrad_partial: unsupported channel counts %d -> %d", cin, cout);
    WgradArgs a;
    a.x1 = (const bf16 *)x1; a.x2 = (const bf16 *)x2; a.C1 = C1; a.C2 = C2; a.g = (const bf16 *)g;
    a.B = B; a.H = H; a.W = W; a.CIN = cin; a.COUT = cout;
    a.partials = partials; a.acc_partials = accumulate;
    return dispatch_wgrad(a, (hipStream_t)stream);
}

extern "C" int mmk_bn_forward_stats(const void *a, int64_t npix, int32_t C, const float *gamma, const float *beta, float eps,
                                    float momentum, float *running_mean, float *running_var, float *part, float *stat, float *affine,
                                    void *stream)
{
    MMK_REQUIRE(a && gamma && beta && part && stat && affine, "mmk_bn_forward_stats: NULL pointer");
    MMK_REQUIRE(npix >= 1 && chan_ok(C) && C <= 2048, "mmk_bn_forward_stats: bad shape (npix %lld, C %d)", (long long)npix, C);
    MMK_REQUIRE((running_mean == nullptr) == (running_var == nullptr), "mmk_bn_forward_stats: running_mean / running_var go together");
    hipStream_t st = (hipStream_t)stream;
    const int per = 256 / (C / 8);
    const int nblk = (int)std::min<int64_t>(BN_BLOCKS, (npix + per - 1) / per);
    hipLaunchKernelGGL(bn_stats_kernel, dim3(nblk), dim3(256), 0, st, (const bf16 *)a, (size_t)npix, C, part);
    MMK_LAUNCH_CHECK();
    hipLaunchKernelGGL(bn_finalize_kernel, dim3((C + 63) / 64), dim3(64), 0, st, part, nblk, C, (double)npix, gamma, beta, eps, momentum,
                       running_mean, running_var, stat, affine);
    MMK_LAUNCH_CHECK();
    return MMK_OK;
}

extern "C" int mmk_bn_apply(const void *a, int64_t npix, int32_t C, const float *affine, float drop_p, uint32_t seed, void *y,
                            void *stream)
{
    MMK_REQUIRE(a && affine && y, "mmk_bn_apply: NULL pointer");
    MMK_REQUIRE(npix >= 1 && chan_ok(C), "mmk_bn_apply: bad shape");
    MMK_REQUIRE(dropout_prob_ok(drop_p), "mmk_bn_apply: dropout probability %g out of range (it is quantised to thr / 65536, thr <= 65535)", (double)drop_p);
    const size_t ngran = (size_t)npix * (C / 8);
    hipLaunchKernelGGL(bn_apply_kernel, dim3((unsigned)std::min<size_t>((ngran + 255) / 256, 8192)), dim3(256), 0, (hipStream_t)stream,
                       (const bf16 *)a, ngran, C, affine, drop_p, seed, (bf16 *)y);
    MMK_LAUNCH_CHECK();
    return MMK_OK;
}

extern "C" int mmk_bn_backward(const void *gd, const void *d, float drop_scale, const void *a, int64_t npix, int32_t C,
                               const float *stat, const float *affine, const float *gamma, float leaky_slope, int32_t accumulate,
                               float *part, float *coef, float *dgamma, float *dbeta, void *gz, void *stream)
{
    MMK_REQUIRE(gd && a && coef && gz, "mmk_bn_backward: NULL pointer");
    MMK_REQUIRE(npix >= 1 && chan_ok(C) && C <= 2048, "mmk_bn_backward: bad shape");
    hipStream_t st = (hipStream_t)stream;
    const size_t ngran = (size_t)npix * (C / 8);
    const unsigned gb = (unsigned)std::min<size_t>((ngran + 255) / 256, 8192);
    if (stat != nullptr) {
        MMK_REQUIRE(gamma && part && dgamma && dbeta, "mmk_bn_backward: NULL pointer (training mode)");
        const int per = 256 / (C / 8);
        const int nblk = (int)std::min<int64_t>(BN_BLOCKS, (npix + per - 1) / per);
        hipLaunchKernelGGL(bn_bwd_reduce_kernel, dim3(nblk), dim3(256), 0, st, (const bf16 *)gd, (const bf16 *)d, drop_scale,
                           (const bf16 *)a, (size_t)npix, C, stat, part);
        MMK_LAUNCH_CHECK();
        hipLaunchKernelGGL(bn_bwd_finalize_kernel, dim3((C + 63) / 64), dim3(64), 0, st, part, nblk, C, (double)npix, gamma, stat,
                           accumulate, coef, dgamma, dbeta);
        MMK_LAUNCH_CHECK();
    } else {
        MMK_REQUIRE(affine != nullptr, "mmk_bn_backward: evaluation mode needs the affine (scale, shift) pairs");
        hipLaunchKernelGGL(bn_eval_coef_kernel, dim3((C + 63) / 64), dim3(64), 0, st, affine, C, coef);
        MMK_LAUNCH_CHECK();
    }
    hipLaunchKernelGGL(bn_bwd_apply_kernel, dim3(gb), dim3(256), 0, st, (const bf16 *)gd, (const bf16 *)d, drop_scale, (const bf16 *)a,
                       ngran, C, stat, coef, leaky_slope, (bf16 *)gz);
    MMK_LAUNCH_CHECK();
    return MMK_OK;
}

static unsigned nblk(size_t n, int t) { return (unsigned)((n + t - 1) / t); }

extern "C" int mmk_channel_minmax(const float *x, int32_t B, int32_t C, int64_t hw, float *part, float *pre, float *minmax,
                                  void *stream)
{
    MMK_REQUIRE(x && part && pre && B >= 1 && C >= 1 && C <= 65535 && hw >= 1, "mmk_channel_minmax: bad argument");
    hipStream_t st = (hipStream_t)stream;
    hipLaunchKernelGGL(channel_minmax_partial_kernel, dim3(MM_BLOCKS, C), dim3(256), 0, st, x, B, C, (size_t)hw, part);
    MMK_LAUNCH_CHECK();
    hipLaunchKernelGGL(channel_minmax_final_kernel, dim3(C), dim3(256), 0, st, part, C, pre, minmax);
    MMK_LAUNCH_CHECK();
    return MMK_OK;
}

extern "C" int mmk_channel_meanstd(const float *x, int32_t B, int32_t C, int64_t hw, double *part, float *pre, void *stream)
{
    MMK_REQUIRE(x && part && pre && B >= 1 && C >= 1 && C <= 65535 && hw >= 1, "mmk_channel_meanstd: bad argument");
    hipStream_t st = (hipStream_t)stream;
    hipLaunchKernelGGL(channel_moment_partial_kernel<false>, dim3(MM_BLOCKS, C), dim3(256), 0, st, x, B, C, (size_t)hw, part);
    MMK_LAUNCH_CHECK();
    hipLaunchKernelGGL(channel_moment_partial_kernel<true>, dim3(MM_BLOCKS, C), dim3(256), 0, st, x, B, C, (size_t)hw, part);
    MMK_LAUNCH_CHECK();
    hipLaunchKernelGGL(channel_meanstd_final_kernel, dim3(C), dim3(256), 0, st, (const double *)part, (size_t)B * (size_t)hw, pre);
    MMK_LAUNCH_CHECK();
    return MMK_OK;
}

extern "C" int mmk_conv_first(const float *x, int32_t cin, const float *W, const float *bias, const float *pre, int32_t B,
                              int32_t H, int32_t Wd, float leaky_slope, void *y, void *stream)
{
    MMK_REQUIRE(x && W && y, "mmk_conv_first: NULL pointer");
    MMK_REQUIRE(leaky_slope >= 0.f && leaky_slope < 1.f, "mmk_conv_first: leaky_slope must be in [0, 1)");
    MMK_REQUIRE(cin >= 1 && cin <= 4 && B >= 1 && H >= 1 && Wd >= 1, "mmk_conv_first: bad shape (cin must be 1..4)");
    const size_t npix = (size_t)B * H * Wd;
    if (Wd % 4 == 0 && npix < (1u << 31)) {
        const unsigned blocks = (unsigned)std::min<size_t>((npix / 4 + 255) / 256, 4096);
        if (leaky_slope > 0.f)
            hipLaunchKernelGGL(conv_first_x4_kernel<true>, dim3(blocks), dim3(256), 0, (hipStream_t)stream, x, cin, W, bias, pre, B, H, Wd,
                               leaky_slope, (bf16 *)y);
        else
            hipLaunchKernelGGL(conv_first_x4_kernel<false>, dim3(blocks), dim3(256), 0, (hipStream_t)stream, x, cin, W, bias, pre, B, H, Wd,
                               leaky_slope, (bf16 *)y);
        MMK_LAUNCH_CHECK();
        return MMK_OK;
    }
    const unsigned blocks = (unsigned)std::min<size_t>((npix + 255) / 256, 8192);
    hipLaunchKernelGGL(conv_first_kernel, dim3(blocks), dim3(256), 0, (hipStream_t)stream, x, cin, W, bias, pre, B, H, Wd, leaky_slope,
                       (bf16 *)y);
    MMK_LAUNCH_CHECK();
    return MMK_OK;
}

extern "C" size_t mmk_conv_first_wgrad_ws_bytes(int32_t cin) { return (size_t)1024 * (cin < 1 ? 1 : cin) * 80 * sizeof(float); }

extern "C" int mmk_conv_first_wgrad(const float *x, int32_t cin, const void *g, const float *pre, int32_t B, int32_t H,
                                    int32_t Wd, float *dW, float *db, float *ws, size_t ws_bytes, void *stream)
{
    MMK_REQUIRE(x && g && dW && ws, "mmk_conv_first_wgrad: NULL pointer");
    MMK_REQUIRE(cin >= 1 && cin <= 4 && B >= 1 && H >= 1 && Wd >= 1, "mmk_conv_first_wgrad: bad shape");
    MMK_REQUIRE(ws_bytes >= mmk_conv_first_wgrad_ws_bytes(cin), "mmk_conv_first_wgrad: workspace too small (%zu < %zu bytes)", ws_bytes,
                mmk_conv_first_wgrad_ws_bytes(cin));
    const size_t npix = (size_t)B * H * Wd;
    unsigned blocks;
    if (Wd % 4 == 0 && npix < (1u << 31)) {
        blocks = (unsigned)std::min<size_t>((npix / 4 + 255) / 256, 512);
        hipLaunchKernelGGL(conv_first_wgrad_x4_kernel, dim3(blocks), dim3(256), 0, (hipStream_t)stream, x, cin, (const bf16 *)g, pre,
                           B, H, Wd, ws);
    } else {
// ... 256 lines not shown
```

mm_masking_amd/csrc/mmk_unet_driver.hip:

```cpp
#include <stdlib.h>
#include <string.h>

#include "mmk_common.h"

namespace {

constexpr int NCONV = 23;
const int ENC_CH[6] = {8, 16, 32, 64, 128, 256};

struct Tens {
    size_t off = 0;
    int h = 0, w = 0, c = 0;
};

struct Plan {
    int B, H, W, cin;
    int rh[6], rw[6];
    int cout[NCONV], cinn[NCONV];
    Tens a_enc[6], d_enc[6], t[6];
    size_t t_arg[6];
    Tens u[5], a1[5], d1[5], a2[5], d2[5];
    size_t packs[NCONV];
    size_t mask_raw, amax, norm_part;
    size_t ws_bytes;
// ... 6 lines not shown
    size_t scratch_bytes;
};

struct Bump {
    size_t off = 0;
    size_t take(size_t bytes)
    {
        off = mmk::align_up(off, 256);
        const size_t o = off;
        off += bytes;
        return o;
    }
    Tens tens(int B, int h, int w, int c)
    {
        Tens t;
        t.h = h; t.w = w; t.c = c;
        t.off = take((size_t)B * h * w * c * 2);
        return t;
    }
};

bool make_plan(Plan &p, int B, int H, int W, int cin, bool with_scratch)
{
    if (B < 1 || H < 32 || W < 32 || cin < 1 || cin > 4) return false;
    p.B = B; p.H = H; p.W = W; p.cin = cin;
    p.rh[0] = H; p.rw[0] = W;
    for (int i = 1; i < 6; ++i) { p.rh[i] = p.rh[i - 1] / 2; p.rw[i] = p.rw[i - 1] / 2; }
    for (int i = 0; i < 6; ++i) {
        p.cinn[2 * i] = i == 0 ? cin : ENC_CH[i - 1]; p.cout[2 * i] = ENC_CH[i];
        p.cinn[2 * i + 1] = ENC_CH[i]; p.cout[2 * i + 1] = ENC_CH[i];
    }
    for (int j = 0; j < 5; ++j) {
        const int cs = ENC_CH[4 - j];
        p.cinn[12 + 2 * j] = 2 * cs; p.cout[12 + 2 * j] = cs;
        p.cinn[13 + 2 * j] = cs; p.cout[13 + 2 * j] = cs;
    }
    p.cinn[22] = 8; p.cout[22] = 1;
    Bump b;
    for (int k = 1; k <= 21; ++k) {
        const size_t n = mmk_conv3x3_packed_elems(p.cout[k], p.cinn[k], 0);
        if (n == 0) return false;
        p.packs[k] = b.take(n * 2);
    }
    p.a_enc[0] = b.tens(B, H, W, 8);
    p.d_enc[0] = b.tens(B, H, W, 8);
    p.t[0] = p.d_enc[0];
    for (int i = 1; i < 6; ++i) {
        p.a_enc[i] = b.tens(B, p.rh[i - 1], p.rw[i - 1], ENC_CH[i]);
        p.d_enc[i] = b.tens(B, p.rh[i - 1], p.rw[i - 1], ENC_CH[i]);
        p.t[i] = b.tens(B, p.rh[i], p.rw[i], ENC_CH[i]);
        p.t_arg[i] = b.take((size_t)B * p.rh[i] * p.rw[i] * ENC_CH[i] / 2);
    }
    for (int j = 0; j < 5; ++j) {
        const int cs = ENC_CH[4 - j], h = p.rh[4 - j], w = p.rw[4 - j];
        p.u[j] = b.tens(B, h, w, 2 * cs);
        p.a1[j] = b.tens(B, h, w, cs);
        p.d1[j] = b.tens(B, h, w, cs);
        p.a2[j] = b.tens(B, h, w, cs);
        p.d2[j] = b.tens(B, h, w, cs);
    }
    p.mask_raw = b.take((size_t)B * H * W * 4);
    p.amax = b.take((size_t)B * 4);
    p.norm_part = b.take((size_t)B * 64 * 4);
    p.ws_bytes = mmk::align_up(b.off, 256);
    if (!with_scratch) return true;

    Bump s;
    for (int k = 1; k <= 21; ++k) p.packs_t[k] = s.take(mmk_conv3x3_packed_elems(p.cout[k], p.cinn[k], 1) * 2);
    p.gz_final = s.tens(B, H, W, 8);
    for (int j = 0; j < 5; ++j) {
        const int cs = ENC_CH[4 - j], h = p.rh[4 - j], w = p.rw[4 - j];
        p.gz_a2[j] = s.tens(B, h, w, cs);
        p.gsk[j] = s.tens(B, h, w, cs);
        p.gz_d1[j] = s.tens(B, h, w, cs);
        p.gz_a1[j] = s.tens(B, h, w, cs);
        p.g_u[j] = s.tens(B, h, w, 2 * cs);
        p.gz_up[j] = s.tens(B, p.rh[5 - j], p.rw[5 - j], 2 * cs);
    }
    for (int i = 1; i < 6; ++i) {
        p.gz_d[i] = s.tens(B, p.rh[i - 1], p.rw[i - 1], ENC_CH[i]);
        p.gz_a[i] = s.tens(B, p.rh[i - 1], p.rw[i - 1], ENC_CH[i]);
    }
    p.gz_a[0] = s.tens(B, H, W, 8);
    for (int k = 1; k <= 21; ++k) {
        int h, w, c1;
        if (k < 12) {
            const int i = k / 2;
            h = i == 0 ? H : p.rh[i - 1]; w = i == 0 ? W : p.rw[i - 1];
            c1 = p.cinn[k];
        } else {
            const int j = (k - 12) / 2;
            h = p.rh[4 - j]; w = p.rw[4 - j];
            c1 = p.cinn[k];
        }
        p.slices[k] = mmk_conv3x3_wgrad_slices(p.cout[k], p.cinn[k], c1, B, h, w);
    }
    for (int k = 1; k <= 21; ++k) {
        if (p.slices[k] <= 0) return false;
        p.part[k] = s.take((size_t)(k >= 12 ? 2 : 1) * p.slices[k] * ((size_t)9 * p.cout[k] * p.cinn[k] + p.cout[k]) * 4);
    }
    p.fin_ws = s.take((size_t)B * 130 * 4);
    p.fin_red = s.take((size_t)MMK_FINAL_BWD_WS_FLOATS * 4);
    p.first_ws = s.take(mmk_conv_first_wgrad_ws_bytes(cin));
    p.scratch_bytes = mmk::align_up(s.off, 256);
    return true;
}

inline void *at(void *base, size_t off) { return static_cast<char *>(base) + off; }

#define MMK_TRY(expr)                \
    do {                             \
        const int rc_ = (expr);      \
        if (rc_ != MMK_OK) return rc_; \
    } while (0)

struct ConvCall {
    const void *x1 = nullptr, *x2 = nullptr;
    int C1 = 0, C2 = 0;
    const void *wpack = nullptr;
    const float *bias = nullptr;
    void *y1 = nullptr, *y2 = nullptr;
    const void *src1 = nullptr, *src2 = nullptr;
    int O1 = 0, O2 = 0, acc1 = 0, acc2 = 0;
    float scale1 = 1.f, scale2 = 1.f;
    int relu = 0;
    float drop_p = 0.f;
    unsigned seed = 0;
    void *pool_y = nullptr, *pool_arg = nullptr;
};

int conv(const Plan &p, int h, int w, float slope, const ConvCall &c, void *stream)
{
    mmk_conv_desc d;
    memset(&d, 0, sizeof(d));
    d.x1 = c.x1; d.x2 = c.x2; d.C1 = c.C1; d.C2 = c.C2; d.wpack = c.wpack; d.bias = c.bias;
    d.y1 = c.y1; d.relu_src1 = c.src1; d.O1 = c.O1; d.accumulate1 = c.acc1; d.scale1 = c.scale1;
    d.y2 = c.y2; d.relu_src2 = c.src2; d.O2 = c.O2; d.accumulate2 = c.acc2; d.scale2 = c.scale2;
    d.B = p.B; d.H = h; d.W = w; d.relu = c.relu; d.leaky_slope = slope; d.drop_p = c.drop_p; d.seed = c.seed;
    d.pool_y = c.pool_y; d.pool_arg = c.pool_arg;
    return mmk_conv3x3(&d, stream);
}

struct SideStream {
    hipStream_t st = nullptr;
    hipEvent_t fork = nullptr, join = nullptr;
    int dev = -1;
};

bool use_side_stream()
{
    static int v = -1;
    if (v < 0) {
        const char *e = getenv("MMK_UNET_SIDE_STREAM");
        v = (e && e[0] == '0') ? 0 : 1;
    }
    return v == 1;
}

int side_stream(SideStream **out)
{
    static thread_local SideStream pool[16];
    int dev = 0;
    MMK_CHECK_HIP(hipGetDevice(&dev));
    SideStream &s = pool[dev & 15];
    if (s.st == nullptr || s.dev != dev) {
        {
            int lo = 0, hi = 0;
            MMK_CHECK_HIP(hipDeviceGetStreamPriorityRange(&lo, &hi));
            MMK_CHECK_HIP(hipStreamCreateWithPriority(&s.st, hipStreamNonBlocking, hi));
        }
        MMK_CHECK_HIP(hipEventCreateWithFlags(&s.fork, hipEventDisableTiming));
        MMK_CHECK_HIP(hipEventCreateWithFlags(&s.join, hipEventDisableTiming));
        s.dev = dev;
    }
    *out = &s;
    return MMK_OK;
}

float dropout_scale(float p)
{
    const unsigned thr = (unsigned)(p * 65536.0f + 0.5f);
    return thr ? 65536.0f / (float)(65536u - thr) : 1.0f;
}

bool dropout_prob_ok(float p) { return p >= 0.f && p < 1.f && (unsigned)(p * 65536.0f + 0.5f) <= 65535u; }

}

extern "C" size_t mmk_unet_workspace_bytes(int32_t B, int32_t H, int32_t W, int32_t cin)
{
    Plan p;
    if (!make_plan(p, B, H, W, cin, false)) {
        mmk::set_error("mmk_unet_workspace_bytes: unsupported network input (B=%d, %d x %d, %d channels)", B, H, W, cin);
        return 0;
    }
    return p.ws_bytes;
}

extern "C" size_t mmk_unet_scratch_bytes(int32_t B, int32_t H, int32_t W, int32_t cin)
{
    Plan p;
    if (!make_plan(p, B, H, W, cin, true)) {
        mmk::set_error("mmk_unet_scratch_bytes: unsupported network input (B=%d, %d x %d, %d channels)", B, H, W, cin);
        return 0;
    }
    return p.scratch_bytes;
}

extern "C" int mmk_unet_tensor(int32_t B, int32_t H, int32_t W, int32_t cin, int32_t id, size_t *offset, int32_t *h, int32_t *w,
                               int32_t *c)
{
    Plan p;
    MMK_REQUIRE(make_plan(p, B, H, W, cin, false), "mmk_unet_tensor: unsupported network input");
    MMK_REQUIRE(offset && h && w && c, "mmk_unet_tensor: NULL pointer");
    const Tens *t = nullptr;
    if (id >= 0 && id < 6) t = &p.a_enc[id];
    else if (id < 12) t = &p.d_enc[id - 6];
    else if (id < 18) t = &p.t[id - 12];
    else if (id < 18 + 25) {
        const int j = (id - 18) / 5, q = (id - 18) % 5;
        const Tens *arr[5] = {&p.u[j], &p.a1[j], &p.d1[j], &p.a2[j], &p.d2[j]};
        t = arr[q];
    }
    MMK_REQUIRE(t != nullptr, "mmk_unet_tensor: bad tensor id %d", id);
    *offset = t->off; *h = t->h; *w = t->w; *c = t->c;
    return MMK_OK;
}

extern "C" int mmk_unet_forward(const mmk_unet_desc *d, void *stream)
{
    MMK_REQUIRE(d != nullptr, "mmk_unet_forward: NULL descriptor");
    MMK_REQUIRE(d->x && d->params && d->workspace && d->mask, "mmk_unet_forward: NULL pointer");
    Plan p;
    MMK_REQUIRE(make_plan(p, d->B, d->H, d->W, d->cin, false), "mmk_unet_forward: unsupported network input (B=%d, %d x %d, %d channels)",
                d->B, d->H, d->W, d->cin);
    MMK_REQUIRE(d->workspace_bytes >= p.ws_bytes, "mmk_unet_forward: workspace too small (%zu < %zu bytes)", d->workspace_bytes,
                p.ws_bytes);
    MMK_REQUIRE(dropout_prob_ok(d->drop_p), "mmk_unet_forward: dropout probability %g out of range (it is quantised to thr / 65536, thr <= 65535)", (double)d->drop_p);
    for (int i = 0; i < 2 * NCONV; ++i) MMK_REQUIRE(d->params[i] != nullptr, "mmk_unet_forward: NULL parameter %d", i);
    void *ws = d->workspace;
    const float sl = d->leaky_slope;
    const int B = p.B;
    auto Wk = [&](int k) { return d->params[2 * k]; };
    auto Bk = [&](int k) { return d->params[2 * k + 1]; };
    unsigned ctr = d->seed * 64u;

    {
        const float *Wp[21];
        void *Op[21];
        int32_t co[21], ci[21];
        for (int k = 1; k <= 21; ++k) {
            Wp[k - 1] = Wk(k); Op[k - 1] = at(ws, p.packs[k]); co[k - 1] = p.cout[k]; ci[k - 1] = p.cinn[k];
        }
        MMK_TRY(mmk_conv3x3_pack_weights_batch(21, Wp, co, ci, 0, Op, stream));
    }
    MMK_TRY(mmk_conv_first(d->x, p.cin, Wk(0), Bk(0), d->pre, B, p.H, p.W, sl, at(ws, p.a_enc[0].off), stream));
    {
        ConvCall c;
        c.x1 = at(ws, p.a_enc[0].off); c.C1 = 8; c.wpack = at(ws, p.packs[1]); c.bias = Bk(1);
        c.y1 = at(ws, p.d_enc[0].off); c.O1 = 8; c.relu = 1; c.drop_p = d->drop_p; c.seed = ++ctr;
        MMK_TRY(conv(p, p.H, p.W, sl, c, stream));
    }
    for (int i = 1; i < 6; ++i) {
        const int h = p.rh[i - 1], w = p.rw[i - 1], ch = ENC_CH[i];
        ConvCall c;
        c.x1 = at(ws, p.t[i - 1].off); c.C1 = ENC_CH[i - 1]; c.wpack = at(ws, p.packs[2 * i]); c.bias = Bk(2 * i);
        c.y1 = at(ws, p.a_enc[i].off); c.O1 = ch; c.relu = 1;
        MMK_TRY(conv(p, h, w, sl, c, stream));
        ConvCall c2;
        c2.x1 = at(ws, p.a_enc[i].off); c2.C1 = ch; c2.wpack = at(ws, p.packs[2 * i + 1]); c2.bias = Bk(2 * i + 1);
        c2.y1 = at(ws, p.d_enc[i].off); c2.O1 = ch; c2.relu = 1; c2.drop_p = d->drop_p; c2.seed = ++ctr;
        const bool fuse = sl == 0.f && mmk_conv3x3_pool_fusable(ch, ch, B, h, w) != 0;
        const bool lean = fuse && !d->keep_full_res;
        if (fuse) c2.pool_y = at(ws, p.t[i].off);
        if (lean) { c2.pool_arg = at(ws, p.t_arg[i]); c2.y1 = nullptr; }
        MMK_TRY(conv(p, h, w, sl, c2, stream));
        if (sl == 0.f) {
            if (!lean) MMK_TRY(mmk_maxpool2_fwd_arg(at(ws, p.d_enc[i].off), B, h, w, ch, at(ws, p.t[i].off), at(ws, p.t_arg[i]), stream));
        } else {
            MMK_TRY(mmk_maxpool2_fwd(at(ws, p.d_enc[i].off), B, h, w, ch, at(ws, p.t[i].off), stream));
        }
    }
    const Tens *cur = &p.t[5];
    for (int j = 0; j < 5; ++j) {
        const int cs = ENC_CH[4 - j], h = p.rh[4 - j], w = p.rw[4 - j];
        const int k0 = 12 + 2 * j, k1 = 13 + 2 * j;
        MMK_TRY(mmk_upsample_fwd(at(ws, cur->off), B, cur->h, cur->w, cur->c, h, w, at(ws, p.u[j].off), stream));
        ConvCall c;
        c.x1 = at(ws, p.u[j].off); c.C1 = 2 * cs; c.wpack = at(ws, p.packs[k0]); c.bias = Bk(k0);
        c.y1 = at(ws, p.a1[j].off); c.O1 = cs; c.relu = 1;
        MMK_TRY(conv(p, h, w, sl, c, stream));
        ConvCall c1;
        c1.x1 = at(ws, p.a1[j].off); c1.C1 = cs; c1.wpack = at(ws, p.packs[k1]); c1.bias = Bk(k1);
        c1.y1 = at(ws, p.d1[j].off); c1.O1 = cs; c1.relu = 1; c1.drop_p = d->drop_p; c1.seed = ++ctr;
        MMK_TRY(conv(p, h, w, sl, c1, stream));
        ConvCall c2;
        c2.x1 = at(ws, p.t[4 - j].off); c2.C1 = cs; c2.x2 = at(ws, p.d1[j].off); c2.C2 = cs;
        c2.wpack = at(ws, p.packs[k0]); c2.bias = Bk(k0); c2.y1 = at(ws, p.a2[j].off); c2.O1 = cs; c2.relu = 1;
        MMK_TRY(conv(p, h, w, sl, c2, stream));
        ConvCall c3;
        c3.x1 = at(ws, p.a2[j].off); c3.C1 = cs; c3.wpack = at(ws, p.packs[k1]); c3.bias = Bk(k1);
        c3.y1 = at(ws, p.d2[j].off); c3.O1 = cs; c3.relu = 1; c3.drop_p = d->drop_p; c3.seed = ++ctr;
        MMK_TRY(conv(p, h, w, sl, c3, stream));
        cur = &p.d2[j];
    }
    float *raw = d->norm ? static_cast<float *>(at(ws, p.mask_raw)) : d->mask;
    MMK_TRY(mmk_final_fwd(at(ws, cur->off), Wk(22), Bk(22), (int64_t)B * p.H * p.W, raw, stream));
    if (d->norm)
        MMK_TRY(mmk_mask_normalize(raw, B, (int64_t)p.H * p.W, static_cast<float *>(at(ws, p.norm_part)), d->mask,
                                   static_cast<float *>(at(ws, p.amax)), stream));
    return MMK_OK;
}

namespace {
struct InputGrad {
    float *grad_x;
    int mode;
    const float *minmax;
};
int unet_backward_impl(const mmk_unet_desc *d, const float *gmask, float *const *grads, void *scratch, size_t scratch_bytes,
                       void *const *bucket_events, void *stream, const InputGrad *ig = nullptr);
}

extern "C" int mmk_unet_backward(const mmk_unet_desc *d, const float *gmask, float *const *grads, void *scratch,
                                 size_t scratch_bytes, void *stream)
{
    return unet_backward_impl(d, gmask, grads, scratch, scratch_bytes, nullptr, stream);
}

extern "C" int32_t mmk_unet_grad_bucket(int32_t bucket, int32_t *first_param, int32_t *n_params)
{
    static const int32_t first[MMK_UNET_GRAD_BUCKETS] = {24, 12, 0}, count[MMK_UNET_GRAD_BUCKETS] = {22, 12, 12};
    MMK_REQUIRE(bucket >= 0 && bucket < MMK_UNET_GRAD_BUCKETS && first_param && n_params, "mmk_unet_grad_bucket: bad bucket %d", bucket);
    *first_param = first[bucket];
    *n_params = count[bucket];
    return MMK_OK;
}

extern "C" int mmk_unet_backward_buckets(const mmk_unet_desc *d, const float *gmask, float *const *grads, void *scratch,
                                         size_t scratch_bytes, void *const *bucket_events, void *stream)
{
    MMK_REQUIRE(bucket_events != nullptr, "mmk_unet_backward_buckets: NULL event array");
    for (int b = 0; b < MMK_UNET_GRAD_BUCKETS; ++b) MMK_REQUIRE(bucket_events[b] != nullptr, "mmk_unet_backward_buckets: NULL event %d", b);
    return unet_backward_impl(d, gmask, grads, scratch, scratch_bytes, bucket_events, stream);
}

extern "C" int mmk_unet_backward_input(const mmk_unet_desc *d, const float *gmask, float *const *grads, float *grad_x,
                                       int32_t norm_mode, const float *minmax, void *scratch, size_t scratch_bytes,
                                       void *const *bucket_events, void *stream)
{
    MMK_REQUIRE(d != nullptr, "mmk_unet_backward_input: NULL descriptor");
    MMK_REQUIRE(grad_x != nullptr, "mmk_unet_backward_input: NULL pointer (grad_x)");
    MMK_REQUIRE(d->cin >= 1 && d->cin <= 4, "mmk_unet_backward_input: bad shape (cin must be 1..4)");
    MMK_REQUIRE(norm_mode == MMK_NORM_NONE || norm_mode == MMK_NORM_MINMAX || norm_mode == MMK_NORM_STANDARDIZE,
                "mmk_unet_backward_input: unknown normalisation mode %d", norm_mode);
    MMK_REQUIRE(norm_mode == MMK_NORM_NONE || d->pre != nullptr, "mmk_unet_backward_input: normalisation mode %d needs d->pre (NULL pointer)",
                norm_mode);
    MMK_REQUIRE(norm_mode != MMK_NORM_MINMAX || minmax != nullptr, "mmk_unet_backward_input: MMK_NORM_MINMAX needs minmax (NULL pointer)");
    MMK_REQUIRE(mmk_conv_first_dgrad_ws_bytes(d->cin) <= mmk_conv_first_wgrad_ws_bytes(d->cin),
                "mmk_unet_backward_input: no room for the statistics in scratch");
    if (bucket_events)
        for (int b = 0; b < MMK_UNET_GRAD_BUCKETS; ++b)
            MMK_REQUIRE(bucket_events[b] != nullptr, "mmk_unet_backward_input: NULL event %d", b);
    const InputGrad ig = {grad_x, norm_mode, norm_mode == MMK_NORM_MINMAX ? minmax : nullptr};
    return unet_backward_impl(d, gmask, grads, scratch, scratch_bytes, bucket_events, stream, &ig);
}

namespace {
int unet_backward_impl(const mmk_unet_desc *d, const float *gmask, float *const *grads, void *scratch, size_t scratch_bytes,
                       void *const *bucket_events, void *stream, const InputGrad *ig)
{
    MMK_REQUIRE(d != nullptr, "mmk_unet_backward: NULL descriptor");
    MMK_REQUIRE(d->x && d->params && d->workspace && d->mask && gmask && grads && scratch, "mmk_unet_backward: NULL pointer");
    Plan p;
    MMK_REQUIRE(make_plan(p, d->B, d->H, d->W, d->cin, true), "mmk_unet_backward: unsupported network input");
    MMK_REQUIRE(d->workspace_bytes >= p.ws_bytes, "mmk_unet_backward: workspace too small");
    MMK_REQUIRE(scratch_bytes >= p.scratch_bytes, "mmk_unet_backward: scratch too small (%zu < %zu bytes)", scratch_bytes, p.scratch_bytes);
    for (int i = 0; i < 2 * NCONV; ++i) MMK_REQUIRE(d->params[i] && grads[i], "mmk_unet_backward: NULL parameter / gradient %d", i);
    void *ws = d->workspace, *sc = scratch;
    hipStream_t st = (hipStream_t)stream;
    const float sl = d->leaky_slope, s = dropout_scale(d->drop_p);
    const int B = p.B;
    auto Wk = [&](int k) { return d->params[2 * k]; };

    {
        const float *Wp[21];
        void *Op[21];
        int32_t co[21], ci[21];
        for (int k = 1; k <= 21; ++k) {
            Wp[k - 1] = Wk(k); Op[k - 1] = at(sc, p.packs_t[k]); co[k - 1] = p.cout[k]; ci[k - 1] = p.cinn[k];
        }
        MMK_TRY(mmk_conv3x3_pack_weights_batch(21, Wp, co, ci, 1, Op, stream));
    }
    SideStream *ss = nullptr;
    if (use_side_stream()) MMK_TRY(side_stream(&ss));
    void *wstream = ss ? (void *)ss->st : stream;
    if (ss) {
        MMK_CHECK_HIP(hipEventRecord(ss->fork, st));
        MMK_CHECK_HIP(hipStreamWaitEvent(ss->st, ss->fork, 0));
    }
    int part_used[NCONV] = {};
    auto part_ptr = [&](int k) {
        float *ptr = static_cast<float *>(at(sc, p.part[k])) +
                     (size_t)part_used[k] * p.slices[k] * ((size_t)9 * p.cout[k] * p.cinn[k] + p.cout[k]);
        part_used[k] += 1;
        return ptr;
    };
    auto unpack = [&](int k0, int k1) -> int {
        if (ss) {
            MMK_CHECK_HIP(hipEventRecord(ss->fork, st));
            MMK_CHECK_HIP(hipStreamWaitEvent(ss->st, ss->fork, 0));
        }
        const float *src[21];
        int32_t slices[21], co[21], ci[21];
        float *dW[21], *db[21];
        int n = 0;
        for (int k = k0; k <= k1; ++k, ++n) {
            src[n] = static_cast<const float *>(at(sc, p.part[k]));
            if (part_used[k] != (k >= 12 ? 2 : 1)) {
                mmk::set_error("mmk_unet_backward: layer %d wrote %d sets of partial slices", k, part_used[k]);
                return MMK_ERR_ARG;
            }
            slices[n] = p.slices[k] * part_used[k]; co[n] = p.cout[k]; ci[n] = p.cinn[k];
            dW[n] = grads[2 * k]; db[n] = grads[2 * k + 1];
        }
        return mmk_conv3x3_wgrad_unpack_batch(n, src, slices, co, ci, dW, db, wstream);
    };

    auto can_fuse = [&](int k, int ch, int h, int w) {
        return (ch == 8 || ch == 16) && sl == 0.f && p.slices[k] > 0 && mmk_conv3x3_wgrad_slices(ch, ch, ch, B, h, w) == p.slices[k];
    };
    auto bwd_fused = [&](int k, int ch, const void *x, const void *g, void *dx, int h, int w) -> int {
        return mmk_conv_bwd_fused(x, g, at(sc, p.packs_t[k]), 1.f, B, h, w, ch, dx, part_ptr(k), 0, stream);
    };
    auto wgrad = [&](int k, const void *x1, int C1, const void *x2, int C2, const void *g, int h, int w) -> int {
        if (ss) {
            MMK_CHECK_HIP(hipEventRecord(ss->fork, st));
            MMK_CHECK_HIP(hipStreamWaitEvent(ss->st, ss->fork, 0));
        }
        if (mmk_conv3x3_wgrad_slices(p.cout[k], p.cinn[k], C1, B, h, w) != p.slices[k]) {
            mmk::set_error("mmk_unet_backward: partial-slice count of layer %d depends on the input split", k);
            return MMK_ERR_ARG;
        }
        return mmk_conv3x3_wgrad_partial(x1, x2, C1, C2, g, p.cout[k], B, h, w, part_ptr(k), 0, wstream);
    };

    const Tens &d2_4 = p.d2[4];
    if (d->norm)
        MMK_TRY(mmk_final_bwd_normalized(at(ws, d2_4.off), Wk(22), static_cast<const float *>(at(ws, p.mask_raw)), d->mask,
                                         static_cast<const float *>(at(ws, p.amax)), gmask, B, (int64_t)p.H * p.W, s, sl,
                                         static_cast<float *>(at(sc, p.fin_ws)), static_cast<float *>(at(sc, p.fin_ws)) + (size_t)B * 128,
                                         at(sc, p.gz_final.off), grads[44], grads[45], static_cast<float *>(at(sc, p.fin_red)), stream));
    else
        MMK_TRY(mmk_final_bwd(at(ws, d2_4.off), Wk(22), d->mask, gmask, (int64_t)B * p.H * p.W, s, sl, at(sc, p.gz_final.off), grads[44],
                              grads[45], static_cast<float *>(at(sc, p.fin_red)), stream));
    const void *gz = at(sc, p.gz_final.off);
    for (int j = 4; j >= 0; --j) {
        const int cs = ENC_CH[4 - j], h = p.rh[4 - j], w = p.rw[4 - j];
        const int k0 = 12 + 2 * j, k1 = 13 + 2 * j;
        const void *skip = at(ws, p.t[4 - j].off);
        const bool fuse8 = can_fuse(k1, cs, h, w);
        if (fuse8) {
            MMK_TRY(bwd_fused(k1, cs, at(ws, p.a2[j].off), gz, at(sc, p.gz_a2[j].off), h, w));
        } else {
            MMK_TRY(wgrad(k1, at(ws, p.a2[j].off), cs, nullptr, 0, gz, h, w));
            ConvCall c;
            c.x1 = gz; c.C1 = cs; c.wpack = at(sc, p.packs_t[k1]); c.y1 = at(sc, p.gz_a2[j].off); c.O1 = cs;
            c.src1 = at(ws, p.a2[j].off); c.scale1 = 1.f;
            MMK_TRY(conv(p, h, w, sl, c, stream));
        }
        if (j == 4 && sl == 0.f && cs == 8 && p.slices[k0] > 0 && mmk_conv3x3_wgrad_slices(8, 16, 8, B, h, w) == p.slices[k0]) {
            MMK_TRY(mmk_conv16x8_bwd_fused(skip, at(ws, p.d1[j].off), at(sc, p.gz_a2[j].off), at(sc, p.packs_t[k0]), s, B, h, w,
                                           at(sc, p.gsk[j].off), at(sc, p.gz_d1[j].off), part_ptr(k0), 0, stream));
        } else {
            MMK_TRY(wgrad(k0, skip, cs, at(ws, p.d1[j].off), cs, at(sc, p.gz_a2[j].off), h, w));
            ConvCall c2;
            c2.x1 = at(sc, p.gz_a2[j].off); c2.C1 = cs; c2.wpack = at(sc, p.packs_t[k0]);
            c2.y1 = at(sc, p.gsk[j].off); c2.O1 = cs; c2.scale1 = s;
            c2.src1 = (j == 4) ? skip : nullptr;
            c2.y2 = at(sc, p.gz_d1[j].off); c2.O2 = cs; c2.src2 = at(ws, p.d1[j].off); c2.scale2 = s;
            MMK_TRY(conv(p, h, w, sl, c2, stream));
        }
        if (fuse8) {
            MMK_TRY(bwd_fused(k1, cs, at(ws, p.a1[j].off), at(sc, p.gz_d1[j].off), at(sc, p.gz_a1[j].off), h, w));
        } else {
            MMK_TRY(wgrad(k1, at(ws, p.a1[j].off), cs, nullptr, 0, at(sc, p.gz_d1[j].off), h, w));
            ConvCall c3;
            c3.x1 = at(sc, p.gz_d1[j].off); c3.C1 = cs; c3.wpack = at(sc, p.packs_t[k1]); c3.y1 = at(sc, p.gz_a1[j].off); c3.O1 = cs;
            c3.src1 = at(ws, p.a1[j].off); c3.scale1 = 1.f;
            MMK_TRY(conv(p, h, w, sl, c3, stream));
        }
        if (j == 4 && sl == 0.f && cs == 8 && p.slices[k0] > 0 && mmk_conv3x3_wgrad_slices(8, 16, 16, B, h, w) == p.slices[k0]) {
            MMK_TRY(mmk_conv16x8_bwd_fused(at(ws, p.u[j].off), nullptr, at(sc, p.gz_a1[j].off), at(sc, p.packs_t[k0]), 1.f, B, h, w,
                                           at(sc, p.g_u[j].off), nullptr, part_ptr(k0), 0, stream));
        } else {
            MMK_TRY(wgrad(k0, at(ws, p.u[j].off), 2 * cs, nullptr, 0, at(sc, p.gz_a1[j].off), h, w));
            ConvCall c4;
            c4.x1 = at(sc, p.gz_a1[j].off); c4.C1 = cs; c4.wpack = at(sc, p.packs_t[k0]); c4.y1 = at(sc, p.g_u[j].off); c4.O1 = 2 * cs;
            MMK_TRY(conv(p, h, w, sl, c4, stream));
        }
        if (j > 0) {
            const Tens &pd2 = p.d2[j - 1];
            MMK_TRY(mmk_upsample_bwd(at(sc, p.g_u[j].off), B, pd2.h, pd2.w, 2 * cs, h, w, at(ws, pd2.off), s, sl, at(sc, p.gz_up[j].off),
                                     stream));
        } else {
            MMK_TRY(mmk_upsample_bwd(at(sc, p.g_u[j].off), B, p.rh[5], p.rw[5], 2 * cs, h, w, nullptr, 1.f, sl, at(sc, p.gz_up[j].off),
                                     stream));
        }
        gz = at(sc, p.gz_up[j].off);
    }
    MMK_TRY(unpack(12, 21));
    if (bucket_events) MMK_CHECK_HIP(hipEventRecord((hipEvent_t)bucket_events[0], (hipStream_t)wstream));
    const void *g_t = gz;
    for (int i = 5; i >= 1; --i) {
        const int ch = ENC_CH[i], h = p.rh[i - 1], w = p.rw[i - 1];
        if (sl == 0.f)
            MMK_TRY(mmk_maxpool2_bwd_arg(at(ws, p.t_arg[i]), g_t, B, h, w, ch, s, at(sc, p.gz_d[i].off), stream));
        else
            MMK_TRY(mmk_maxpool2_bwd(at(ws, p.d_enc[i].off), g_t, B, h, w, ch, s, sl, at(sc, p.gz_d[i].off), stream));
        if (can_fuse(2 * i + 1, ch, h, w)) {
            MMK_TRY(bwd_fused(2 * i + 1, ch, at(ws, p.a_enc[i].off), at(sc, p.gz_d[i].off), at(sc, p.gz_a[i].off), h, w));
        } else {
            MMK_TRY(wgrad(2 * i + 1, at(ws, p.a_enc[i].off), ch, nullptr, 0, at(sc, p.gz_d[i].off), h, w));
            ConvCall c;
            c.x1 = at(sc, p.gz_d[i].off); c.C1 = ch; c.wpack = at(sc, p.packs_t[2 * i + 1]); c.y1 = at(sc, p.gz_a[i].off); c.O1 = ch;
            c.src1 = at(ws, p.a_enc[i].off); c.scale1 = 1.f;
            MMK_TRY(conv(p, h, w, sl, c, stream));
        }
        void *tgt = at(sc, p.gsk[5 - i].off);
        if (i == 1 && sl == 0.f && ch == 16 && ENC_CH[0] == 8 && p.slices[2] > 0 &&
            mmk_conv3x3_wgrad_slices(16, 8, 8, B, h, w) == p.slices[2]) {
            MMK_TRY(mmk_conv8x16_bwd_fused(at(ws, p.t[0].off), at(sc, p.gz_a[1].off), at(sc, p.packs_t[2]), s, B, h, w, tgt,
                                           part_ptr(2), 0, stream));
        } else {
            MMK_TRY(wgrad(2 * i, at(ws, p.t[i - 1].off), ENC_CH[i - 1], nullptr, 0, at(sc, p.gz_a[i].off), h, w));
            ConvCall c2;
            c2.x1 = at(sc, p.gz_a[i].off); c2.C1 = ch; c2.wpack = at(sc, p.packs_t[2 * i]); c2.y1 = tgt; c2.O1 = ENC_CH[i - 1];
            c2.acc1 = 1;
            if (i == 1) { c2.src1 = at(ws, p.t[0].off); c2.scale1 = s; }
            MMK_TRY(conv(p, h, w, sl, c2, stream));
        }
        g_t = tgt;
        if (i == 3) {
            MMK_TRY(unpack(6, 11));
            if (bucket_events) MMK_CHECK_HIP(hipEventRecord((hipEvent_t)bucket_events[1], (hipStream_t)wstream));
        }
    }
    if (can_fuse(1, 8, p.H, p.W)) {
        MMK_TRY(bwd_fused(1, 8, at(ws, p.a_enc[0].off), g_t, at(sc, p.gz_a[0].off), p.H, p.W));
    } else {
        MMK_TRY(wgrad(1, at(ws, p.a_enc[0].off), 8, nullptr, 0, g_t, p.H, p.W));
        ConvCall c;
        c.x1 = g_t; c.C1 = 8; c.wpack = at(sc, p.packs_t[1]); c.y1 = at(sc, p.gz_a[0].off); c.O1 = 8;
        c.src1 = at(ws, p.a_enc[0].off); c.scale1 = 1.f;
        MMK_TRY(conv(p, p.H, p.W, sl, c, stream));
    }
    MMK_TRY(unpack(1, 5));
    MMK_TRY(mmk_conv_first_wgrad(d->x, p.cin, at(sc, p.gz_a[0].off), d->pre, B, p.H, p.W, grads[0], grads[1],
                                 static_cast<float *>(at(sc, p.first_ws)), mmk_conv_first_wgrad_ws_bytes(p.cin), stream));
    if (ss) {
        MMK_CHECK_HIP(hipEventRecord(ss->join, ss->st));
        MMK_CHECK_HIP(hipStreamWaitEvent(st, ss->join, 0));
    }
    if (bucket_events) MMK_CHECK_HIP(hipEventRecord((hipEvent_t)bucket_events[2], st));
    if (ig) {
        const size_t nws = mmk_conv_first_dgrad_ws_bytes(p.cin);
        void *sws = ig->mode == MMK_NORM_NONE ? nullptr : at(sc, p.first_ws);
        MMK_TRY(mmk_conv_first_dgrad(at(sc, p.gz_a[0].off), p.cin, Wk(0), d->x, d->pre, ig->minmax, B, p.H, p.W, ig->grad_x, sws, nws,
                                     stream));
        MMK_TRY(mmk_input_norm_bwd(ig->grad_x, d->x, p.cin, d->pre, ig->minmax, ig->mode, B, p.H, p.W, sws, nws, stream));
    }
    return MMK_OK;
}
}
```

mm_masking_amd/unet_hip.py:

```python
import ctypes
import os

import torch

from . import _lib

BF16 = torch.bfloat16


def _p(t):
    return None if t is None else ctypes.c_void_p(t.data_ptr())


def pack_weights(w, transposed=False):
    L = _lib.lib()
    cout, cin = w.shape[0], w.shape[1]
    n = L.mmk_conv3x3_packed_elems(cout, cin, 1 if transposed else 0)
    if n == 0:
        raise _lib.MmkError("unsupported conv channel counts %d -> %d" % (cin, cout))
    out = torch.empty(n, dtype=BF16, device=w.device)
    wf = w.detach().float().contiguous()
    _lib.check(L.mmk_conv3x3_pack_weights(_lib.ptr(wf), cout, cin, 1 if transposed else 0, _lib.ptr(out),
                                          _lib.stream_ptr(w.device)))
    return out


def pack_weights_batch(ws, transposed=False):
    L = _lib.lib()
    n = len(ws)
    tr = 1 if transposed else 0
    sizes = [L.mmk_conv3x3_packed_elems(w.shape[0], w.shape[1], tr) for w in ws]
    if any(sz == 0 for sz in sizes):
        raise _lib.MmkError("unsupported conv channel counts in pack_weights_batch")
    offs = [0]
    for sz in sizes:
        offs.append(offs[-1] + (sz + 127) // 128 * 128)
    buf = torch.empty(offs[-1], dtype=BF16, device=ws[0].device)
    base = buf.data_ptr()
    wsrc = [w.detach().float().contiguous() for w in ws]
    Wp = (ctypes.c_void_p * n)(*[w.data_ptr() for w in wsrc])
    Op = (ctypes.c_void_p * n)(*[base + 2 * o for o in offs[:-1]])
    co = (ctypes.c_int32 * n)(*[w.shape[0] for w in ws])
    ci = (ctypes.c_int32 * n)(*[w.shape[1] for w in ws])
    _lib.check(L.mmk_conv3x3_pack_weights_batch(n, Wp, co, ci, tr, Op, _lib.stream_ptr(ws[0].device)))
    return [buf[offs[i]:offs[i] + sizes[i]] for i in range(n)]


def conv3x3(x1, wpack, cout, bias=None, x2=None, relu=False, drop_p=0.0, seed=0, out=None, out2=None, split=None,
            relu_src=None, scale=1.0, relu_src2=None, scale2=1.0, accumulate=False, accumulate2=False, pool_out=None,
            slope=0.0, pool_arg=None):
    B, H, W, C1 = x1.shape
    C2 = 0 if x2 is None else x2.shape[3]
    O1 = cout if split is None else split
    O2 = cout - O1
    if out is None and pool_arg is None:
        out = torch.empty(B, H, W, O1, dtype=BF16, device=x1.device)
    if O2 > 0 and out2 is None:
        out2 = torch.empty(B, H, W, O2, dtype=BF16, device=x1.device)
    d = _lib.ConvDesc(x1=_p(x1), x2=_p(x2), C1=C1, C2=C2, wpack=_p(wpack), bias=_p(bias), y1=_p(out),
                      relu_src1=_p(relu_src), O1=O1, accumulate1=1 if accumulate else 0, scale1=float(scale),
                      y2=_p(out2), relu_src2=_p(relu_src2), O2=O2, accumulate2=1 if accumulate2 else 0,
                      scale2=float(scale2), B=B, H=H, W=W, relu=1 if relu else 0, leaky_slope=float(slope),
                      drop_p=float(drop_p),
                      seed=int(seed) & 0xFFFFFFFF, pool_y=_p(pool_out), pool_arg=_p(pool_arg))
    _lib.check(_lib.lib().mmk_conv3x3(ctypes.byref(d), _lib.stream_ptr(x1.device)))
    if pool_arg is not None:
        return None
    return (out, out2) if O2 > 0 else out


def pool_fusable(cin, cout, B, H, W):
    return bool(_lib.lib().mmk_conv3x3_pool_fusable(cin, cout, B, H, W))


def conv3x3_wgrad(x1, g, cout, x2=None, dWt=None, db=None):
    B, H, W, C1 = x1.shape
    C2 = 0 if x2 is None else x2.shape[3]
    cin = C1 + C2
    ns = wgrad_slices(cout, cin, C1, B, H, W)
    if ns <= 0:
        raise _lib.MmkError("conv3x3_wgrad: unsupported shape %d -> %d channels" % (cin, cout))
    part = partial_buffer(ns, cout, cin, x1.device)
    conv3x3_wgrad_partial(x1, g, cout, part, x2=x2)
    tot = part.sum(dim=0)
    w = tot[:9 * cout * cin].view(9, cout, cin)
    if dWt is None:
        dWt = w.clone()
    else:
        dWt += w
    if db is not None:
        db += tot[9 * cout * cin:]
    return dWt


def wgrad_unpack(dWt, accumulate_into=None):
    w = dWt.permute(1, 2, 0).reshape(dWt.shape[1], dWt.shape[2], 3, 3)
    if accumulate_into is not None:
        accumulate_into += w
        return accumulate_into
    return w.contiguous()


def dropout_scale(p):
    f32 = lambda v: ctypes.c_float(v).value
    thr = int(f32(f32(float(p)) * 65536.0 + 0.5))
    return 65536.0 / (65536 - thr) if thr else 1.0


def wgrad_slices(cout, cin, c1, B, H, W):
    return int(_lib.lib().mmk_conv3x3_wgrad_slices(cout, cin, c1, B, H, W))


def partial_buffer(ns, cout, cin, device):
    return torch.empty(ns, 9 * cout * cin + cout, dtype=torch.float32, device=device)


def conv3x3_wgrad_partial(x1, g, cout, partials, x2=None, accumulate=False):
    B, H, W, C1 = x1.shape
    C2 = 0 if x2 is None else x2.shape[3]
    _lib.check(_lib.lib().mmk_conv3x3_wgrad_partial(_p(x1), _p(x2), C1, C2, _p(g), cout, B, H, W, _p(partials),
                                                    1 if accumulate else 0, _lib.stream_ptr(x1.device)))
    return partials


def conv_bwd_fused(x, g, wpack_t, scale, dx, partials, accumulate=False):
    B, H, W, C = x.shape
    assert C in (8, 16) and g.shape == x.shape and dx.shape == x.shape
    _lib.check(_lib.lib().mmk_conv_bwd_fused(_p(x), _p(g), _p(wpack_t), float(scale), B, H, W, C, _p(dx), _p(partials),
                                             1 if accumulate else 0, _lib.stream_ptr(x.device)))
    return dx, partials


def conv8x16_bwd_fused(x, g, wpack_t, scale, dx, partials, accumulate=False):
    B, H, W, C = x.shape
    assert C == 8 and g.shape == (B, H, W, 16) and dx.shape == x.shape
    _lib.check(_lib.lib().mmk_conv8x16_bwd_fused(_p(x), _p(g), _p(wpack_t), float(scale), B, H, W, _p(dx), _p(partials),
                                                 1 if accumulate else 0, _lib.stream_ptr(x.device)))
    return dx, partials


def conv16x8_bwd_fused(x1, x2, g, wpack_t, scale, dx1, dx2, partials, accumulate=False):
    B, H, W, C = x1.shape
    if x2 is None:
        assert C == 16 and dx2 is None and g.shape == (B, H, W, 8) and dx1.shape == x1.shape
    else:
        assert C == 8 and x2.shape == x1.shape and g.shape == x1.shape and dx1.shape == x1.shape and dx2.shape == x1.shape
    _lib.check(_lib.lib().mmk_conv16x8_bwd_fused(_p(x1), _p(x2), _p(g), _p(wpack_t), float(scale), B, H, W, _p(dx1), _p(dx2),
                                                 _p(partials), 1 if accumulate else 0, _lib.stream_ptr(x1.device)))
    return dx1, dx2, partials


def wgrad_unpack_batch(items):
    n = len(items)
    srcs, couts, cins, slices, dbs = [], [], [], [], []
    for it in items:
        if isinstance(it, (tuple, list)):
            t, co, ci = it[0], it[1], it[2]
            srcs.append(t); couts.append(co); cins.append(ci); slices.append(t.shape[0])
            dbs.append(it[3] if len(it) > 3 else None)
        else:
            srcs.append(it); couts.append(it.shape[1]); cins.append(it.shape[2]); slices.append(0); dbs.append(None)
    sizes = [9 * co * ci for co, ci in zip(couts, cins)]
    offs = [0]
    for sz in sizes:
        offs.append(offs[-1] + (sz + 3) // 4 * 4)
    dev = srcs[0].device
    buf = torch.empty(offs[-1], dtype=torch.float32, device=dev)
    base = buf.data_ptr()
    Sp = (ctypes.c_void_p * n)(*[t.data_ptr() for t in srcs])
    Op = (ctypes.c_void_p * n)(*[base + 4 * o for o in offs[:-1]])
    Dp = (ctypes.c_void_p * n)(*[(d.data_ptr() if d is not None else None) for d in dbs])
    sl = (ctypes.c_int32 * n)(*slices)
    co = (ctypes.c_int32 * n)(*couts)
    ci = (ctypes.c_int32 * n)(*cins)
    _lib.check(_lib.lib().mmk_conv3x3_wgrad_unpack_batch(n, Sp, sl, co, ci, Op, Dp, _lib.stream_ptr(dev)))
    return [buf[offs[i]:offs[i] + sizes[i]].view(couts[i], cins[i], 3, 3) for i in range(n)]


def _sp(dev):
    return _lib.stream_ptr(dev)


def conv_first_wgrad(x, gz, pre, dW, db):
    L = _lib.lib()
    B, cin, H, W = x.shape
    nb = int(L.mmk_conv_first_wgrad_ws_bytes(cin))
    ws = torch.empty(nb // 4, dtype=torch.float32, device=x.device)
    _lib.check(L.mmk_conv_first_wgrad(_p(x), cin, _p(gz), _p(pre), B, H, W, _p(dW), _p(db), _p(ws), nb, _sp(x.device)))


def conv_first_dgrad(gz, w, x=None, pre=None, minmax=None, stats=False):
    L = _lib.lib()
    B, H, W, _ = gz.shape
    cin = w.shape[1]
    gx = torch.empty(B, cin, H, W, dtype=torch.float32, device=gz.device)
    ws, nb = None, 0
    if stats:
        nb = int(L.mmk_conv_first_dgrad_ws_bytes(cin))
        ws = torch.empty(nb // 8, dtype=torch.float64, device=gz.device)
    _lib.check(L.mmk_conv_first_dgrad(_p(gz), cin, _p(w), _p(x), _p(pre), _p(minmax), B, H, W, _p(gx), _p(ws), nb, _sp(gz.device)))
    return gx, ws


def input_norm_bwd(gx, x, pre, mode, minmax, ws):
    B, cin, H, W = gx.shape
    _lib.check(_lib.lib().mmk_input_norm_bwd(_p(gx), _p(x), cin, _p(pre), _p(minmax), _lib.NORM_MODES[mode], B, H, W, _p(ws),
                                             0 if ws is None else ws.numel() * 8, _sp(gx.device)))
    return gx


def first_layer_input_grad(x, gz, w, pre, in_norm):
    mode, mm = in_norm if in_norm is not None else (None, None)
    if _lib.NORM_MODES[mode] == 0:
        return conv_first_dgrad(gz, w, pre=pre)[0]
    gx, ws = conv_first_dgrad(gz, w, x=x, pre=pre, minmax=mm if mode == "minmax" else None, stats=True)
    return input_norm_bwd(gx, x, pre, mode, mm, ws)


def conv_first(x, w, b, pre=None, slope=0.0):
    B, cin, H, W = x.shape
    y = torch.empty(B, H, W, 8, dtype=BF16, device=x.device)
    _lib.check(_lib.lib().mmk_conv_first(_p(x), cin, _p(w), _p(b), _p(pre), B, H, W, float(slope), _p(y), _sp(x.device)))
    return y


FORCE_COLLECTIVES = False


def minmax_is_collective(global_reduce, process_group=None):
    import torch.distributed as dist
    return bool(global_reduce and dist.is_available() and dist.is_initialized()
                and (dist.get_world_size(process_group) > 1 or FORCE_COLLECTIVES))


def channel_minmax(x, process_group=None, global_reduce=False, return_minmax=False):
    B, C, H, W = x.shape
    part = torch.empty(C * 2048, dtype=torch.float32, device=x.device)
    pre = torch.empty(C, 2, dtype=torch.float32, device=x.device)
    import torch.distributed as dist
    reduce = minmax_is_collective(global_reduce, process_group)
    mm = torch.empty(C, 2, dtype=torch.float32, device=x.device) if (reduce or return_minmax) else None
    _lib.check(_lib.lib().mmk_channel_minmax(_p(x), B, C, H * W, _p(part), _p(pre), _p(mm), _sp(x.device)))
    if reduce:
        t = torch.stack((-mm[:, 0], mm[:, 1]), dim=1)
        dist.all_reduce(t, op=dist.ReduceOp.MAX, group=process_group)
        pre = torch.stack((-t[:, 0], 1.0 / (t[:, 1] + t[:, 0])), dim=1).contiguous()
    return (pre, mm) if return_minmax else pre


def channel_meanstd(x):
    B, C, H, W = x.shape
    part = torch.empty(C * 2048, dtype=torch.float64, device=x.device)
    pre = torch.empty(C, 2, dtype=torch.float32, device=x.device)
    _lib.check(_lib.lib().mmk_channel_meanstd(_p(x), B, C, H * W, _p(part), _p(pre), _sp(x.device)))
    return pre


def maxpool2(x):
    B, H, W, C = x.shape
    y = torch.empty(B, H // 2, W // 2, C, dtype=BF16, device=x.device)
    _lib.check(_lib.lib().mmk_maxpool2_fwd(_p(x), B, H, W, C, _p(y), _sp(x.device)))
    return y


def maxpool2_arg(x):
    B, H, W, C = x.shape
    y = torch.empty(B, H // 2, W // 2, C, dtype=BF16, device=x.device)
    arg = torch.empty(B, H // 2, W // 2, C // 2, dtype=torch.uint8, device=x.device)
    _lib.check(_lib.lib().mmk_maxpool2_fwd_arg(_p(x), B, H, W, C, _p(y), _p(arg), _sp(x.device)))
    return y, arg


def maxpool2_bwd_arg(arg, gy, H, W, scale):
    B, _, _, C = gy.shape
    gz = torch.empty(B, H, W, C, dtype=BF16, device=gy.device)
    _lib.check(_lib.lib().mmk_maxpool2_bwd_arg(_p(arg), _p(gy), B, H, W, C, float(scale), _p(gz), _sp(gy.device)))
    return gz


def maxpool2_bwd(d, gy, scale, slope=0.0):
    B, H, W, C = d.shape
    gz = torch.empty_like(d)
    _lib.check(_lib.lib().mmk_maxpool2_bwd(_p(d), _p(gy), B, H, W, C, float(scale), float(slope), _p(gz), _sp(d.device)))
    return gz


def upsample(x, Ho, Wo):
    B, Hs, Ws, C = x.shape
    y = torch.empty(B, Ho, Wo, C, dtype=BF16, device=x.device)
    _lib.check(_lib.lib().mmk_upsample_fwd(_p(x), B, Hs, Ws, C, Ho, Wo, _p(y), _sp(x.device)))
    return y


def upsample_bwd(gy, Hs, Ws, relu_src=None, scale=1.0, slope=0.0):
    B, Ho, Wo, C = gy.shape
    gx = torch.empty(B, Hs, Ws, C, dtype=BF16, device=gy.device)
    _lib.check(_lib.lib().mmk_upsample_bwd(_p(gy), B, Hs, Ws, C, Ho, Wo, _p(relu_src), float(scale), float(slope),
                                           _p(gx), _sp(gy.device)))
    return gx


# ... 343 lines not shown
```

Baseline: 3396 pairs/s.

## Extend fused conv backward (dgrad+wgrad) kernel to 32-channel layers

Generalizes the fused backward conv kernel, which computes input gradient and weight-gradient partials in one pass over shared x/g tiles, to layers with 32 channels. It uses dynamic LDS with padded pitches for the larger tiles. The driver routes the 32/16-channel encoder and decoder layers through the new 16x32 and 32x16 variants instead of separate wgrad and dgrad conv launches. This saves a second read of activations and gradients plus extra launches, at the cost of higher LDS and register use per block, which may reduce occupancy.

```diff
diff --git a/include/mmk.h b/include/mmk.h
--- a/include/mmk.h
+++ b/include/mmk.h
@@ -248,6 +248,12 @@
 
 int mmk_conv16x8_bwd_fused(const void *x1, const void *x2, const void *g, const void *wpack_t, float scale, int32_t B, int32_t H,
                            int32_t W, void *dx1, void *dx2, float *partials, int32_t accumulate, void *stream);
+
+int mmk_conv16x32_bwd_fused(const void *x, const void *g, const void *wpack_t, float scale, int32_t masked, int32_t B, int32_t H,
+                            int32_t W, void *dx, float *partials, int32_t accumulate, void *stream);
+int mmk_conv32x16_bwd_fused(const void *x1, const void *x2, const void *g, const void *wpack_t, float scale, int32_t mask_x1,
+                            int32_t B, int32_t H, int32_t W, void *dx1, void *dx2, float *partials, int32_t accumulate,
+                            void *stream);
 int mmk_conv3x3_wgrad_unpack_batch(int32_t n, const float *const *src, const int32_t *slices, const int32_t *cout,
                                    const int32_t *cin, float *const *dW, float *const *db, void *stream);
 
diff --git a/mm_masking_amd/_lib.py b/mm_masking_amd/_lib.py
--- a/mm_masking_amd/_lib.py
+++ b/mm_masking_amd/_lib.py
@@ -143,6 +143,9 @@
         "mmk_conv_bwd_fused": (ctypes.c_int, [c_vp, c_vp, c_vp, ctypes.c_float, i32, i32, i32, i32, c_vp, c_vp, i32, c_vp]),
         "mmk_conv8x16_bwd_fused": (ctypes.c_int, [c_vp, c_vp, c_vp, ctypes.c_float, i32, i32, i32, c_vp, c_vp, i32, c_vp]),
         "mmk_conv16x8_bwd_fused": (ctypes.c_int, [c_vp, c_vp, c_vp, c_vp, ctypes.c_float, i32, i32, i32, c_vp, c_vp, c_vp, i32, c_vp]),
+        "mmk_conv16x32_bwd_fused": (ctypes.c_int, [c_vp, c_vp, c_vp, ctypes.c_float, i32, i32, i32, i32, c_vp, c_vp, i32, c_vp]),
+        "mmk_conv32x16_bwd_fused": (ctypes.c_int, [c_vp, c_vp, c_vp, c_vp, ctypes.c_float, i32, i32, i32, i32, c_vp, c_vp, c_vp, i32,
+                                                   c_vp]),
         "mmk_conv3x3_pool_fusable": (ctypes.c_int32, [i32, i32, i32, i32, i32]),
         "mmk_channel_minmax": (ctypes.c_int, [c_vp, i32, i32, ctypes.c_int64, c_vp, c_vp, c_vp, c_vp]),
         "mmk_channel_meanstd": (ctypes.c_int, [c_vp, i32, i32, ctypes.c_int64, c_vp, c_vp, c_vp]),
diff --git a/mm_masking_amd/csrc/mmk_unet.hip b/mm_masking_amd/csrc/mmk_unet.hip
--- a/mm_masking_amd/csrc/mmk_unet.hip
+++ b/mm_masking_amd/csrc/mmk_unet.hip
@@ -1595,18 +1595,38 @@
     int acc_partials;
 };
 
+__host__ __device__ constexpr bool bwd_fused_dyn(int cx, int cg) { return cx == 32 || cg == 32; }
+__host__ __device__ constexpr size_t bwd_fused_lds_bytes(int cx, int cg)
+{
+    return ((size_t)(HT * WT + 8) * (lds_pitch(cx) + lds_pitch(cg)) + (size_t)ksteps(cg) * (cx == 32 ? 2 : 1) * 512) * sizeof(bf16);
+}
+
 template <int CX, int CG>
 __global__ __launch_bounds__(CONV_THREADS) void conv_bwd_fused_kernel(const BwdFusedArgs a)
 {
-    static_assert((CX == 8 || CX == 16) && (CG == 8 || CG == 16), "thin layers");
-    constexpr int NTT = CX == 8 ? 5 : 9;
+    static_assert((CX == 8 || CX == 16 || CX == 32) && (CG == 8 || CG == 16 || CG == 32), "thin layers");
+    constexpr int XT = CX == 32 ? 2 : 1;
+    constexpr int GT = CG == 32 ? 2 : 1;
+    constexpr int NTT = CX == 8 ? 5 : 9 * XT;
     constexpr int NTW = (NTT + 3) / 4;
-    constexpr int NS = CG == 8 ? 3 : 5;
+    constexpr int NS = ksteps(CG);
     constexpr int NT = 4;
     constexpr int GX = CX / 8, GG = CG / 8;
-    __shared__ __attribute__((aligned(16))) bf16 x_tile[(HT * WT + 8) * CX];
-    __shared__ __attribute__((aligned(16))) bf16 g_tile[(HT * WT + 8) * CG];
-    __shared__ __attribute__((aligned(16))) bf16 w_lds[NS * 64 * 8];
+    constexpr int PX = lds_pitch(CX), PG = lds_pitch(CG);
+    constexpr bool DYN = bwd_fused_dyn(CX, CG);
+    constexpr bool ACC = CX == 16 && CG == 32;
+    bf16 *x_tile, *g_tile, *w_lds;
+    if constexpr (DYN) {
+        extern __shared__ __attribute__((aligned(16))) unsigned char smem[];
+        x_tile = reinterpret_cast<bf16 *>(smem);
+        g_tile = x_tile + (HT * WT + 8) * PX;
+        w_lds = g_tile + (HT * WT + 8) * PG;
+    } else {
+        __shared__ __attribute__((aligned(16))) bf16 x_stat[(HT * WT + 8) * CX];
+        __shared__ __attribute__((aligned(16))) bf16 g_stat[(HT * WT + 8) * CG];
+        __shared__ __attribute__((aligned(16))) bf16 w_stat[NS * 64 * 8];
+        x_tile = x_stat; g_tile = g_stat; w_lds = w_stat;
+    }
 
     const int tid = threadIdx.x, lane = tid & 63;
     const int wv = __builtin_amdgcn_readfirstlane(tid >> 6);
@@ -1616,9 +1636,13 @@
     const int i16 = lane & 15, g4 = lane >> 4, q = i16 >> 2, pp = i16 & 3;
     const bool split = a.x2 != nullptr;
 
-    f32x4 acc[NTW], accb = {0.f, 0.f, 0.f, 0.f};
-#pragma unroll
-    for (int n = 0; n < NTW; ++n) acc[n] = (f32x4){0.f, 0.f, 0.f, 0.f};
+    f32x4 acc[GT][NTW], accb[GT];
+#pragma unroll
+    for (int m = 0; m < GT; ++m) {
+        accb[m] = (f32x4){0.f, 0.f, 0.f, 0.f};
+#pragma unroll
+        for (int n = 0; n < NTW; ++n) acc[m][n] = (f32x4){0.f, 0.f, 0.f, 0.f};
+    }
     bf16x8 ones;
 #pragma unroll
     for (int j = 0; j < 8; ++j) ones[j] = (bf16)1.0f;
@@ -1626,21 +1650,21 @@
 #pragma unroll
     for (int n = 0; n < NTW; ++n) {
         const int nt = wv + 4 * n;
-        int tap = CX == 8 ? 2 * nt + (pp >> 1) : nt;
-        const int col = CX == 8 ? 4 * (pp & 1) : 4 * pp;
+        int tap = CX == 8 ? 2 * nt + (pp >> 1) : nt / XT;
+        const int col = CX == 8 ? 4 * (pp & 1) : (nt % XT) * 16 + 4 * pp;
         tap = tap > 8 ? 8 : tap;
         const int ty = tap / 3, tx = tap % 3;
-        b_ad[n] = lds_addr(x_tile) + (unsigned)((((ty * WT) + 4 * g4 + q + tx) * CX + col) * 2);
-    }
-    const unsigned g_ad = lds_addr(g_tile) + (unsigned)(((WT + 1 + 4 * g4 + q) * CG + 4 * pp) * 2);
+        b_ad[n] = lds_addr(x_tile) + (unsigned)((((ty * WT) + 4 * g4 + q + tx) * PX + col) * 2);
+    }
+    const unsigned g_ad = lds_addr(g_tile) + (unsigned)(((WT + 1 + 4 * g4 + q) * PG + 4 * pp) * 2);
 
     int d_lane[NS];
 #pragma unroll
     for (int ks = 0; ks < NS; ++ks) {
-        int tap = CG == 8 ? 4 * ks + (lane >> 4) : 2 * ks + (lane >> 5);
-        const int ch = CG == 8 ? 0 : 8 * ((lane >> 4) & 1);
+        int tap = CG == 8 ? 4 * ks + (lane >> 4) : (CG == 16 ? 2 * ks + (lane >> 5) : ks);
+        const int ch = CG == 8 ? 0 : (CG == 16 ? 8 * ((lane >> 4) & 1) : 8 * (lane >> 4));
         tap = tap > 8 ? 8 : tap;
-        d_lane[ks] = ((2 * wv + tap / 3) * WT + (lane & 15) + tap % 3) * CG + ch;
+        d_lane[ks] = ((2 * wv + tap / 3) * WT + (lane & 15) + tap % 3) * PG + ch;
     }
     const int n8 = lane >> 4;
     const int lrow8 = 2 * wv + (n8 >> 1), lcol8 = (n8 & 1) * 16 + (lane & 15);
@@ -1651,14 +1675,21 @@
     for (int n = 0; n < NT; ++n) {
         const int r = 2 * wv + (n >> 1), c = (n & 1) * 16 + (lane & 15);
         o_pix[n] = r * a.W + c;
-        s_off[n] = ((r + 1) * WT + c + 1) * CX + (lane >> 4) * 4;
-    }
-    bf16 *const o_base = (a.dx2 != nullptr) ? ((lane >> 5) ? a.dx2 : a.dx) + ((lane >> 4) & 1) * 4 : a.dx + (lane >> 4) * 4;
-    const int o_stride = (a.dx2 != nullptr) ? 8 : 16;
-    for (int i = tid; i < NS * 64; i += CONV_THREADS) reinterpret_cast<u32x4 *>(w_lds)[i] = reinterpret_cast<const u32x4 *>(a.wpack_t)[i];
+        s_off[n] = ((r + 1) * WT + c + 1) * PX + (lane >> 4) * 4;
+    }
+    bf16 *o_base[XT];
+    if constexpr (CX == 32) {
+        o_base[0] = a.dx + (lane >> 4) * 4;
+        o_base[1] = ((a.dx2 != nullptr) ? a.dx2 : a.dx + 16) + (lane >> 4) * 4;
+    } else {
+        o_base[0] = (a.dx2 != nullptr) ? ((lane >> 5) ? a.dx2 : a.dx) + ((lane >> 4) & 1) * 4 : a.dx + (lane >> 4) * 4;
+    }
+    const int o_stride = (a.dx2 != nullptr) ? (CX == 32 ? 16 : 8) : (CX == 32 ? 32 : 16);
+    for (int i = tid; i < NS * XT * 64; i += CONV_THREADS) reinterpret_cast<u32x4 *>(w_lds)[i] = reinterpret_cast<const u32x4 *>(a.wpack_t)[i];
 
     constexpr int NX = HT * WT * GX, NG = HT * WT * GG;
     constexpr int RX = (NX + CONV_THREADS - 1) / CONV_THREADS, RG = (NG + CONV_THREADS - 1) / CONV_THREADS;
+    constexpr int HX = CX == 32 ? 2 : 1, HC = CX == 32 ? 16 : 8;
     u32x4 rx[RX], rg[RG];
     auto load_tile = [&](int b, int tyi, int txi) {
         int tv = tid;
@@ -1669,11 +1700,11 @@
         for (int i = 0; i < RX; ++i) {
             int gi = tv + i * CONV_THREADS;
             gi = gi < NX ? gi : NX - 1;
-            const int pix = gi / GX, half = gi % GX;
+            const int pix = gi / GX, gc = gi % GX;
             const int dy = pix / WT - 1, dx = pix % WT - 1;
             const bool ok = (unsigned)(ty0 + dy) < (unsigned)a.H && (unsigned)(tx0 + dx) < (unsigned)a.W;
             const long po = pix0 + dy * a.W + dx;
-            const bf16 *src = split ? (half ? a.x2 : a.x) + po * 8 : a.x + po * CX + half * 8;
+            const bf16 *src = split ? ((gc / HX) ? a.x2 : a.x) + po * HC + (gc % HX) * 8 : a.x + po * CX + gc * 8;
             rx[i] = *(ok ? reinterpret_cast<const u32x4 *>(src) : &g_zero16);
         }
 #pragma unroll
@@ -1692,12 +1723,12 @@
 #pragma unroll
         for (int i = 0; i < RX; ++i) {
             const int gi = tv + i * CONV_THREADS;
-            if (gi < NX) *reinterpret_cast<u32x4 *>(x_tile + (size_t)gi * 8) = rx[i];
+            if (gi < NX) *reinterpret_cast<u32x4 *>(x_tile + (PX == CX ? (size_t)gi * 8 : (size_t)(gi / GX) * PX + (gi % GX) * 8)) = rx[i];
         }
 #pragma unroll
         for (int i = 0; i < RG; ++i) {
             const int gi = tv + i * CONV_THREADS;
-            if (gi < NG) *reinterpret_cast<u32x4 *>(g_tile + (size_t)gi * 8) = rg[i];
+            if (gi < NG) *reinterpret_cast<u32x4 *>(g_tile + (PG == CG ? (size_t)gi * 8 : (size_t)(gi / GG) * PG + (gi % GG) * 8)) = rg[i];
         }
     };
 
@@ -1726,6 +1757,15 @@
         const bool ok8 = (ty0 + lrow8) < a.H && (tx0 + lcol8) < a.W;
         u32x4 e8_acc = {0u, 0u, 0u, 0u};
         if constexpr (CX == 8) e8_acc = *((ok8 && a.accumulate_dx) ? reinterpret_cast<const u32x4 *>(a.dx + (long)(pix0 + lpix8) * 8) : &g_zero16);
+        bf16x4 e_acc[ACC ? NT : 1];
+        if constexpr (ACC) {
+#pragma unroll
+            for (int n = 0; n < NT; ++n) {
+                const bool okp = (ty0 + 2 * wv + (n >> 1)) < a.H && (tx0 + (n & 1) * 16 + (lane & 15)) < a.W;
+                e_acc[n] = *((okp && a.accumulate_dx) ? reinterpret_cast<const bf16x4 *>(o_base[0] + (long)(pix0 + o_pix[n]) * o_stride)
+                                                      : reinterpret_cast<const bf16x4 *>(&g_zero16));
+            }
+        }
         {
             if (t + t_step < t_end) {
                 ld_tx += adv_tx;
@@ -1739,22 +1779,28 @@
             load_tile(ld_b, ld_ty, ld_tx);
             cb = ld_b; cty = ld_ty; ctx = ld_tx;
         }
-        i32x2 fa[2][2], fb[2][2 * NTW];
+        i32x2 fa[2][2 * GT], fb[2][2 * NTW];
 #define BF_ISSUE(R, BUF)                                                                     \
     {                                                                                        \
-        fa[BUF][0] = tr_read_o<((R) * WT * CG) * 2>(g_ad);                                   \
-        fa[BUF][1] = tr_read_o<((R) * WT * CG + 16 * CG) * 2>(g_ad);                         \
+        _Pragma("unroll") for (int m = 0; m < GT; ++m) {                                     \
+            fa[BUF][2 * m] = (m == 0) ? tr_read_o<((R) * WT * PG) * 2>(g_ad)                 \
+                                      : tr_read_o<((R) * WT * PG + 16) * 2>(g_ad);           \
+            fa[BUF][2 * m + 1] = (m == 0) ? tr_read_o<((R) * WT * PG + 16 * PG) * 2>(g_ad)   \
+                                          : tr_read_o<((R) * WT * PG + 16 + 16 * PG) * 2>(g_ad); \
+        }                                                                                    \
         _Pragma("unroll") for (int n = 0; n < NTW; ++n) {                                    \
-            fb[BUF][2 * n] = tr_read_o<((R) * WT * CX) * 2>(b_ad[n]);                        \
-            fb[BUF][2 * n + 1] = tr_read_o<((R) * WT * CX + 16 * CX) * 2>(b_ad[n]);          \
+            fb[BUF][2 * n] = tr_read_o<((R) * WT * PX) * 2>(b_ad[n]);                        \
+            fb[BUF][2 * n + 1] = tr_read_o<((R) * WT * PX + 16 * PX) * 2>(b_ad[n]);          \
         }                                                                                    \
     }
 #define BF_CONSUME(BUF)                                                                      \
     {                                                                                        \
-        const bf16x8 af = frag_from(fa[BUF][0], fa[BUF][1]);                                 \
-        _Pragma("unroll") for (int n = 0; n < NTW; ++n)                                      \
-            acc[n] = __builtin_amdgcn_mfma_f32_16x16x32_bf16(af, frag_from(fb[BUF][2 * n], fb[BUF][2 * n + 1]), acc[n], 0, 0, 0); \
-        accb = __builtin_amdgcn_mfma_f32_16x16x32_bf16(af, ones, accb, 0, 0, 0);             \
+        _Pragma("unroll") for (int m = 0; m < GT; ++m) {                                     \
+            const bf16x8 af = frag_from(fa[BUF][2 * m], fa[BUF][2 * m + 1]);                 \
+            _Pragma("unroll") for (int n = 0; n < NTW; ++n)                                  \
+                acc[m][n] = __builtin_amdgcn_mfma_f32_16x16x32_bf16(af, frag_from(fb[BUF][2 * n], fb[BUF][2 * n + 1]), acc[m][n], 0, 0, 0); \
+            accb[m] = __builtin_amdgcn_mfma_f32_16x16x32_bf16(af, ones, accb[m], 0, 0, 0);   \
+        }                                                                                    \
     }
 #define BF_STEP(R)                                                                           \
     {                                                                                        \
@@ -1770,26 +1816,33 @@
 #undef BF_STEP
 #undef BF_CONSUME
 #undef BF_ISSUE
-        f32x4 dacc[NT];
-#pragma unroll
-        for (int n = 0; n < NT; ++n) dacc[n] = (f32x4){0.f, 0.f, 0.f, 0.f};
+        f32x4 dacc[XT][NT];
+#pragma unroll
+        for (int m = 0; m < XT; ++m)
+#pragma unroll
+            for (int n = 0; n < NT; ++n) dacc[m][n] = (f32x4){0.f, 0.f, 0.f, 0.f};
 #pragma unroll
         for (int ks = 0; ks < NS; ++ks) {
-            const bf16 *bl = g_tile + d_lane[ks];
+            const bf16 *bl = g_tile + (CG == 32 ? d_lane[0] + ((ks / 3) * WT + ks % 3) * PG : d_lane[ks]);
             bf16x8 bf[NT];
 #pragma unroll
-            for (int n = 0; n < NT; ++n) bf[n] = *reinterpret_cast<const bf16x8 *>(bl + ((n >> 1) * WT + (n & 1) * 16) * CG);
-            const bf16x8 af = *reinterpret_cast<const bf16x8 *>(w_lds + ((size_t)(ks * 64 + lane)) * 8);
-#pragma unroll
-            for (int n = 0; n < NT; ++n) dacc[n] = __builtin_amdgcn_mfma_f32_16x16x32_bf16(af, bf[n], dacc[n], 0, 0, 0);
+            for (int n = 0; n < NT; ++n) bf[n] = *reinterpret_cast<const bf16x8 *>(bl + ((n >> 1) * WT + (n & 1) * 16) * PG);
+#pragma unroll
+            for (int m = 0; m < XT; ++m) {
+                const bf16x8 af = *reinterpret_cast<const bf16x8 *>(w_lds + ((size_t)((ks * XT + m) * 64 + lane)) * 8);
+#pragma unroll
+                for (int n = 0; n < NT; ++n) dacc[m][n] = __builtin_amdgcn_mfma_f32_16x16x32_bf16(af, bf[n], dacc[m][n], 0, 0, 0);
+            }
         }
         u32x4 e8_src = {0u, 0u, 0u, 0u};
-        bf16x4 e_src[NT];
+        bf16x4 e_src[XT][NT];
         if constexpr (CX == 8) {
             e8_src = *reinterpret_cast<const u32x4 *>(x_tile + s_off8);
         } else {
 #pragma unroll
-            for (int n = 0; n < NT; ++n) e_src[n] = *reinterpret_cast<const bf16x4 *>(x_tile + s_off[n]);
+            for (int m = 0; m < XT; ++m)
+#pragma unroll
+                for (int n = 0; n < NT; ++n) e_src[m][n] = *reinterpret_cast<const bf16x4 *>(x_tile + s_off[n] + m * 16);
         }
 #pragma unroll
         for (int i = 0; i < RX; ++i) asm volatile("" : "+v"(rx[i]));
@@ -1799,8 +1852,8 @@
             float v8[8];
 #pragma unroll
             for (int r = 0; r < 4; ++r) {
-                const auto s01 = __builtin_amdgcn_permlane16_swap(__float_as_uint(dacc[0][r]), __float_as_uint(dacc[1][r]), false, false);
-                const auto s23 = __builtin_amdgcn_permlane16_swap(__float_as_uint(dacc[2][r]), __float_as_uint(dacc[3][r]), false, false);
+                const auto s01 = __builtin_amdgcn_permlane16_swap(__float_as_uint(dacc[0][0][r]), __float_as_uint(dacc[0][1][r]), false, false);
+                const auto s23 = __builtin_amdgcn_permlane16_swap(__float_as_uint(dacc[0][2][r]), __float_as_uint(dacc[0][3][r]), false, false);
                 const auto lo = __builtin_amdgcn_permlane32_swap(s01[0], s23[0], false, false);
                 const auto hi = __builtin_amdgcn_permlane32_swap(s01[1], s23[1], false, false);
                 v8[r] = __uint_as_float(lo[0]);
@@ -1821,15 +1874,20 @@
 #pragma unroll
             for (int n = 0; n < NT; ++n) {
                 const bool okp = (ty0 + 2 * wv + (n >> 1)) < a.H && (tx0 + (n & 1) * 16 + (lane & 15)) < a.W;
-                bf16x4 outv;
-#pragma unroll
-                for (int r = 0; r < 4; ++r) {
-                    const float v = fmaxf(dacc[n][r] + 0.f, -INFINITY);
-                    const float masked = ((float)e_src[n][r] > 0.f) ? v * a.scale : 0.f;
-                    outv[r] = (bf16)(a.masked ? masked + 0.f : v);
+#pragma unroll
+                for (int m = 0; m < XT; ++m) {
+                    const bool mk = (CX == 32) ? ((a.masked >> ((a.dx2 != nullptr) ? m : 0)) & 1) != 0 : a.masked != 0;
+                    bf16x4 outv;
+#pragma unroll
+                    for (int r = 0; r < 4; ++r) {
+                        const float v = fmaxf(dacc[m][n][r] + 0.f, -INFINITY);
+                        const float masked = ((float)e_src[m][n][r] > 0.f) ? v * a.scale : 0.f;
+                        if constexpr (ACC) outv[r] = (bf16)((mk ? masked : v) + (float)e_acc[n][r]);
+                        else outv[r] = (bf16)(mk ? masked + 0.f : v);
+                    }
+                    bf16x4 *dst = okp ? reinterpret_cast<bf16x4 *>(o_base[m] + (long)(pix0 + o_pix[n]) * o_stride) : reinterpret_cast<bf16x4 *>(g_sink16);
+                    *dst = outv;
                 }
-                bf16x4 *dst = okp ? reinterpret_cast<bf16x4 *>(o_base + (long)(pix0 + o_pix[n]) * o_stride) : reinterpret_cast<bf16x4 *>(g_sink16);
-                *dst = outv;
             }
         }
         if (t + t_step >= t_end) break;
@@ -1840,23 +1898,26 @@
 
     constexpr size_t pstride = (size_t)9 * CG * CX + CG;
 #pragma unroll
-    for (int rr = 0; rr < 4; ++rr) {
-        const int co = g4 * 4 + rr;
-        if (co >= CG) continue;
-#pragma unroll
-        for (int n = 0; n < NTW; ++n) {
-            const int nt = wv + 4 * n;
-            if (nt >= NTT) continue;
-            const int tap = CX == 8 ? 2 * nt + (i16 >> 3) : nt;
-            const int ci = CX == 8 ? (i16 & 7) : i16;
-            if (tap < 9) {
-                float *d = a.partials + (size_t)blockIdx.x * pstride + ((size_t)tap * CG + co) * CX + ci;
-                *d = a.acc_partials ? *d + acc[n][rr] : acc[n][rr];
-            }
-        }
-        if (wv == 0 && i16 == 0) {
-            float *d = a.partials + (size_t)blockIdx.x * pstride + (size_t)9 * CG * CX + co;
-            *d = a.acc_partials ? *d + accb[rr] : accb[rr];
+    for (int m = 0; m < GT; ++m) {
+#pragma unroll
+        for (int rr = 0; rr < 4; ++rr) {
+            const int co = m * 16 + g4 * 4 + rr;
+            if (co >= CG) continue;
+#pragma unroll
+            for (int n = 0; n < NTW; ++n) {
+                const int nt = wv + 4 * n;
+                if (nt >= NTT) continue;
+                const int tap = CX == 8 ? 2 * nt + (i16 >> 3) : nt / XT;
+                const int ci = CX == 8 ? (i16 & 7) : (nt % XT) * 16 + i16;
+                if (tap < 9) {
+                    float *d = a.partials + (size_t)blockIdx.x * pstride + ((size_t)tap * CG + co) * CX + ci;
+                    *d = a.acc_partials ? *d + acc[m][n][rr] : acc[m][n][rr];
+                }
+            }
+            if (wv == 0 && i16 == 0) {
+                float *d = a.partials + (size_t)blockIdx.x * pstride + (size_t)9 * CG * CX + co;
+                *d = a.acc_partials ? *d + accb[m][rr] : accb[m][rr];
+            }
         }
     }
 }
@@ -3631,7 +3692,17 @@
         mmk::set_error("fused backward: occupancy query failed");
         return MMK_ERR_HIP;
     }
-    hipLaunchKernelGGL((conv_bwd_fused_kernel<CX, CG>), dim3(spatial), dim3(CONV_THREADS), 0, st, a);
+    constexpr size_t smem = bwd_fused_dyn(CX, CG) ? bwd_fused_lds_bytes(CX, CG) : 0;
+    if constexpr (smem > 64 * 1024) {
+        static bool attr_set[64] = {};
+        int dev = 0;
+        MMK_CHECK_HIP(hipGetDevice(&dev));
+        if (!attr_set[dev & 63]) {
+            MMK_CHECK_HIP(hipFuncSetAttribute((const void *)conv_bwd_fused_kernel<CX, CG>, hipFuncAttributeMaxDynamicSharedMemorySize, (int)smem));
+            attr_set[dev & 63] = true;
+        }
+    }
+    hipLaunchKernelGGL((conv_bwd_fused_kernel<CX, CG>), dim3(spatial), dim3(CONV_THREADS), smem, st, a);
     MMK_LAUNCH_CHECK();
     return MMK_OK;
 }
@@ -3640,11 +3711,12 @@
                                   int32_t C, void *dx, float *partials, int32_t accumulate, void *stream)
 {
     MMK_REQUIRE(x && g && wpack_t && dx && partials, "mmk_conv_bwd_fused: NULL pointer");
-    MMK_REQUIRE(B >= 1 && H >= 2 && W >= 2 && (C == 8 || C == 16), "mmk_conv_bwd_fused: bad shape (8 or 16 channels)");
+    MMK_REQUIRE(B >= 1 && H >= 2 && W >= 2 && (C == 8 || C == 16 || C == 32), "mmk_conv_bwd_fused: bad shape (8, 16 or 32 channels)");
     MMK_REQUIRE((size_t)B * H * W * C < ((size_t)1 << 31), "mmk_conv_bwd_fused: tensor too large for 32-bit offsets");
     BwdFusedArgs a = {};
     a.x = (const bf16 *)x; a.g = (const bf16 *)g; a.wpack_t = (const bf16 *)wpack_t; a.dx = (bf16 *)dx; a.scale = scale; a.masked = 1;
     a.B = B; a.H = H; a.W = W; a.partials = partials; a.acc_partials = accumulate;
+    if (C == 32) return launch_bwd_fused<32, 32>(a, 32, (hipStream_t)stream);
     return C == 8 ? launch_bwd_fused<8, 8>(a, 8, (hipStream_t)stream) : launch_bwd_fused<16, 16>(a, 16, (hipStream_t)stream);
 }
 
@@ -3673,6 +3745,35 @@
     a.dx = (bf16 *)dx1; a.dx2 = (bf16 *)dx2; a.scale = scale; a.masked = x2 != nullptr;
     a.B = B; a.H = H; a.W = W; a.partials = partials; a.acc_partials = accumulate;
     return launch_bwd_fused<16, 8>(a, x2 ? 8 : 16, (hipStream_t)stream);
+}
+
+extern "C" int mmk_conv16x32_bwd_fused(const void *x, const void *g, const void *wpack_t, float scale, int32_t masked, int32_t B, int32_t H,
+                                       int32_t W, void *dx, float *partials, int32_t accumulate, void *stream)
+{
+    MMK_REQUIRE(x && g && wpack_t && dx && partials, "mmk_conv16x32_bwd_fused: NULL pointer");
+    MMK_REQUIRE(B >= 1 && H >= 2 && W >= 2, "mmk_conv16x32_bwd_fused: bad shape");
+    MMK_REQUIRE((size_t)B * H * W * 32 < ((size_t)1 << 31), "mmk_conv16x32_bwd_fused: tensor too large for 32-bit offsets");
+    BwdFusedArgs a = {};
+    a.x = (const bf16 *)x; a.g = (const bf16 *)g; a.wpack_t = (const bf16 *)wpack_t; a.dx = (bf16 *)dx; a.scale = scale;
+    a.masked = masked != 0; a.accumulate_dx = 1;
+    a.B = B; a.H = H; a.W = W; a.partials = partials; a.acc_partials = accumulate;
+    return launch_bwd_fused<16, 32>(a, 16, (hipStream_t)stream);
+}
+
+extern "C" int mmk_conv32x16_bwd_fused(const void *x1, const void *x2, const void *g, const void *wpack_t, float scale, int32_t mask_x1,
+                                       int32_t B, int32_t H, int32_t W, void *dx1, void *dx2, float *partials, int32_t accumulate,
+                                       void *stream)
+{
+    MMK_REQUIRE(x1 && g && wpack_t && dx1 && partials, "mmk_conv32x16_bwd_fused: NULL pointer");
+    MMK_REQUIRE((x2 == nullptr) == (dx2 == nullptr), "mmk_conv32x16_bwd_fused: x2 and dx2 go together (both NULL: one 32-channel input / unmasked output)");
+    MMK_REQUIRE(B >= 1 && H >= 2 && W >= 2, "mmk_conv32x16_bwd_fused: bad shape");
+    MMK_REQUIRE((size_t)B * H * W * 32 < ((size_t)1 << 31), "mmk_conv32x16_bwd_fused: tensor too large for 32-bit offsets");
+    BwdFusedArgs a = {};
+    a.x = (const bf16 *)x1; a.x2 = (const bf16 *)x2; a.g = (const bf16 *)g; a.wpack_t = (const bf16 *)wpack_t;
+    a.dx = (bf16 *)dx1; a.dx2 = (bf16 *)dx2; a.scale = scale;
+    a.masked = x2 ? ((mask_x1 != 0) ? 3 : 2) : 0;
+    a.B = B; a.H = H; a.W = W; a.partials = partials; a.acc_partials = accumulate;
+    return launch_bwd_fused<32, 16>(a, x2 ? 16 : 32, (hipStream_t)stream);
 }
 
 extern "C" int32_t mmk_conv3x3_wgrad_slices(int32_t cout, int32_t cin, int32_t c1, int32_t B, int32_t H, int32_t W)
diff --git a/mm_masking_amd/csrc/mmk_unet_driver.hip b/mm_masking_amd/csrc/mmk_unet_driver.hip
--- a/mm_masking_amd/csrc/mmk_unet_driver.hip
+++ b/mm_masking_amd/csrc/mmk_unet_driver.hip
@@ -182,6 +182,16 @@
     static int v = -1;
     if (v < 0) {
         const char *e = getenv("MMK_UNET_SIDE_STREAM");
+        v = (e && e[0] == '0') ? 0 : 1;
+    }
+    return v == 1;
+}
+
+bool use_bwd_fused32()
+{
+    static int v = -1;
+    if (v < 0) {
+        const char *e = getenv("MMK_BWD_FUSED32");
         v = (e && e[0] == '0') ? 0 : 1;
     }
     return v == 1;
@@ -457,8 +467,10 @@
         return mmk_conv3x3_wgrad_unpack_batch(n, src, slices, co, ci, dW, db, wstream);
     };
 
+    const bool fused32 = use_bwd_fused32();
     auto can_fuse = [&](int k, int ch, int h, int w) {
-        return (ch == 8 || ch == 16) && sl == 0.f && p.slices[k] > 0 && mmk_conv3x3_wgrad_slices(ch, ch, ch, B, h, w) == p.slices[k];
+        return (ch == 8 || ch == 16 || (ch == 32 && fused32)) && sl == 0.f && p.slices[k] > 0 &&
+               mmk_conv3x3_wgrad_slices(ch, ch, ch, B, h, w) == p.slices[k];
     };
     auto bwd_fused = [&](int k, int ch, const void *x, const void *g, void *dx, int h, int w) -> int {
         return mmk_conv_bwd_fused(x, g, at(sc, p.packs_t[k]), 1.f, B, h, w, ch, dx, part_ptr(k), 0, stream);
@@ -502,6 +514,10 @@
         if (j == 4 && sl == 0.f && cs == 8 && p.slices[k0] > 0 && mmk_conv3x3_wgrad_slices(8, 16, 8, B, h, w) == p.slices[k0]) {
             MMK_TRY(mmk_conv16x8_bwd_fused(skip, at(ws, p.d1[j].off), at(sc, p.gz_a2[j].off), at(sc, p.packs_t[k0]), s, B, h, w,
                                            at(sc, p.gsk[j].off), at(sc, p.gz_d1[j].off), part_ptr(k0), 0, stream));
+        } else if (j == 3 && fused32 && sl == 0.f && cs == 16 && p.slices[k0] > 0 &&
+                   mmk_conv3x3_wgrad_slices(16, 32, 16, B, h, w) == p.slices[k0]) {
+            MMK_TRY(mmk_conv32x16_bwd_fused(skip, at(ws, p.d1[j].off), at(sc, p.gz_a2[j].off), at(sc, p.packs_t[k0]), s, 0, B, h, w,
+                                            at(sc, p.gsk[j].off), at(sc, p.gz_d1[j].off), part_ptr(k0), 0, stream));
         } else {
             MMK_TRY(wgrad(k0, skip, cs, at(ws, p.d1[j].off), cs, at(sc, p.gz_a2[j].off), h, w));
             ConvCall c2;
@@ -523,6 +539,10 @@
         if (j == 4 && sl == 0.f && cs == 8 && p.slices[k0] > 0 && mmk_conv3x3_wgrad_slices(8, 16, 16, B, h, w) == p.slices[k0]) {
             MMK_TRY(mmk_conv16x8_bwd_fused(at(ws, p.u[j].off), nullptr, at(sc, p.gz_a1[j].off), at(sc, p.packs_t[k0]), 1.f, B, h, w,
                                            at(sc, p.g_u[j].off), nullptr, part_ptr(k0), 0, stream));
+        } else if (j == 3 && fused32 && sl == 0.f && cs == 16 && p.slices[k0] > 0 &&
+                   mmk_conv3x3_wgrad_slices(16, 32, 32, B, h, w) == p.slices[k0]) {
+            MMK_TRY(mmk_conv32x16_bwd_fused(at(ws, p.u[j].off), nullptr, at(sc, p.gz_a1[j].off), at(sc, p.packs_t[k0]), 1.f, 0, B, h, w,
+                                            at(sc, p.g_u[j].off), nullptr, part_ptr(k0), 0, stream));
         } else {
             MMK_TRY(wgrad(k0, at(ws, p.u[j].off), 2 * cs, nullptr, 0, at(sc, p.gz_a1[j].off), h, w));
             ConvCall c4;
@@ -562,6 +582,10 @@
             mmk_conv3x3_wgrad_slices(16, 8, 8, B, h, w) == p.slices[2]) {
             MMK_TRY(mmk_conv8x16_bwd_fused(at(ws, p.t[0].off), at(sc, p.gz_a[1].off), at(sc, p.packs_t[2]), s, B, h, w, tgt,
                                            part_ptr(2), 0, stream));
+        } else if (i == 2 && fused32 && sl == 0.f && ch == 32 && ENC_CH[1] == 16 && p.slices[4] > 0 &&
+                   mmk_conv3x3_wgrad_slices(32, 16, 16, B, h, w) == p.slices[4]) {
+            MMK_TRY(mmk_conv16x32_bwd_fused(at(ws, p.t[1].off), at(sc, p.gz_a[2].off), at(sc, p.packs_t[4]), 1.f, 0, B, h, w, tgt,
+                                            part_ptr(4), 0, stream));
         } else {
             MMK_TRY(wgrad(2 * i, at(ws, p.t[i - 1].off), ENC_CH[i - 1], nullptr, 0, at(sc, p.gz_a[i].off), h, w));
             ConvCall c2;
diff --git a/mm_masking_amd/unet_hip.py b/mm_masking_amd/unet_hip.py
--- a/mm_masking_amd/unet_hip.py
+++ b/mm_masking_amd/unet_hip.py
@@ -125,7 +125,7 @@
 
 def conv_bwd_fused(x, g, wpack_t, scale, dx, partials, accumulate=False):
     B, H, W, C = x.shape
-    assert C in (8, 16) and g.shape == x.shape and dx.shape == x.shape
+    assert C in (8, 16, 32) and g.shape == x.shape and dx.shape == x.shape
     _lib.check(_lib.lib().mmk_conv_bwd_fused(_p(x), _p(g), _p(wpack_t), float(scale), B, H, W, C, _p(dx), _p(partials),
                                              1 if accumulate else 0, _lib.stream_ptr(x.device)))
     return dx, partials
@@ -147,6 +147,25 @@
         assert C == 8 and x2.shape == x1.shape and g.shape == x1.shape and dx1.shape == x1.shape and dx2.shape == x1.shape
     _lib.check(_lib.lib().mmk_conv16x8_bwd_fused(_p(x1), _p(x2), _p(g), _p(wpack_t), float(scale), B, H, W, _p(dx1), _p(dx2),
                                                  _p(partials), 1 if accumulate else 0, _lib.stream_ptr(x1.device)))
+    return dx1, dx2, partials
+
+
+def conv16x32_bwd_fused(x, g, wpack_t, scale, dx, partials, masked=True, accumulate=False):
+    B, H, W, C = x.shape
+    assert C == 16 and g.shape == (B, H, W, 32) and dx.shape == x.shape
+    _lib.check(_lib.lib().mmk_conv16x32_bwd_fused(_p(x), _p(g), _p(wpack_t), float(scale), 1 if masked else 0, B, H, W, _p(dx),
+                                                  _p(partials), 1 if accumulate else 0, _lib.stream_ptr(x.device)))
+    return dx, partials
+
+
+def conv32x16_bwd_fused(x1, x2, g, wpack_t, scale, dx1, dx2, partials, mask_x1=True, accumulate=False):
+    B, H, W, C = x1.shape
+    if x2 is None:
+        assert C == 32 and dx2 is None and g.shape == (B, H, W, 16) and dx1.shape == x1.shape
+    else:
+        assert C == 16 and x2.shape == x1.shape and g.shape == x1.shape and dx1.shape == x1.shape and dx2.shape == x1.shape
+    _lib.check(_lib.lib().mmk_conv32x16_bwd_fused(_p(x1), _p(x2), _p(g), _p(wpack_t), float(scale), 1 if mask_x1 else 0, B, H, W,
+                                                  _p(dx1), _p(dx2), _p(partials), 1 if accumulate else 0, _lib.stream_ptr(x1.device)))
     return dx1, dx2, partials
 
 
```

Result: no change. 3389 pairs/s (-0.2%).
